# jafarinia/snuffy

Hardware: AMD Instinct MI355X
Metric: slides/sec (higher is better)
Workload: dtype f32; 1 GPU; cfgB: MILNet eval forward, 1 bag/step/rank, N=32768 patches D=768 h=6 Lambda=200 (K=200) depth=1 relu mlp x4; parallelism=bag-parallel x1, bags_resident_per_rank=8, launch=hip graph replay, rccl_ranks=0

## Files before the change

include/snuffy_hip.h:

```cpp
#ifndef SNUFFY_HIP_H
#define SNUFFY_HIP_H

#include <stddef.h>
#include <stdint.h>

#ifdef __cplusplus
extern "C" {
#endif

typedef void* snf_stream_t;

#define SNF_OK 0
#define SNF_EINVAL (-1)
#define SNF_ELAUNCH (-2)
#define SNF_EUNSUPPORTED (-3)
#define SNF_EWORKSPACE (-4)

#define SNF_ACT_RELU 0
#define SNF_ACT_GELU 1
#define SNF_ACT_LEAKYRELU 2
#define SNF_ACT_SELU 3
#define SNF_ACT_NONE 4

#define SNF_DT_F32 0
// ... 3 lines not shown

const char* snf_version(void);
const char* snf_last_error(void);
int snf_device_cu_count(void);

int snf_critic_f32(const float* x, int64_t n, int d, const float* w, const float* b, int c_out, float* scores,
                   float* colmax_val, int64_t* colmax_idx, snf_stream_t stream);
int snf_critic_ln_f32(const float* x, int64_t n, int d, const float* w, const float* b, int c_out, float* scores,
                      float eps, void* xhat_bf16, snf_stream_t stream);

#define SNF_TOPK_MAX_K 2048
size_t snf_topk_workspace_bytes(int64_t n, int k);
int snf_topk_f32(const float* scores, int64_t n, int64_t stride, int k, int64_t* idx_out, void* workspace,
                 size_t workspace_bytes, snf_stream_t stream);
int snf_topk_gather_f32(const float* scores, int64_t n, int64_t stride, int k, int64_t* idx_out, const float* x,
                        int d, float* xs, void* workspace, size_t workspace_bytes, snf_stream_t stream);
int snf_gather_rows_f32(const float* x, int64_t n, int d, const int64_t* idx, int k, float* out,
                        snf_stream_t stream);

size_t snf_selector_state_bytes(void);
int snf_critic_select_f32(const float* x, int64_t n, int d, const float* w, const float* b, float* scores, float eps,
                          void* xhat_bf16, void* selector_state, snf_stream_t stream);
int snf_topk_select_f32(const float* scores, int64_t n, int k, int64_t* idx_out, void* selector_state,
                        snf_stream_t stream);
int snf_topk_hist_select_f32(const float* scores, int64_t n, int64_t stride, int k, int64_t* idx_out, void* state,
                             snf_stream_t stream);

int snf_scatter_rows_f32(const float* x, int64_t n, int d, const int64_t* idx, int k, const float* rows, float* y,
                         snf_stream_t stream);
int snf_scatter_add_rows_f32(float* z, int64_t n, int d, const int64_t* idx, int k, const float* delta,
                             snf_stream_t stream);
int snf_slot_map_i32(const int64_t* idx, int k, int64_t n, int32_t* map, snf_stream_t stream);
int snf_gather_slot_map_f32(const float* x, int64_t n, int d, const int64_t* idx, int k, float* xs, int32_t* map,
                            void* xs_bf16, snf_stream_t stream);

int snf_layernorm_rows_f32(const float* x, int64_t n, int d, const int32_t* slot_map, const float* patch_rows,
                           const float* gamma, const float* beta, float eps, float* out_f32, void* out_bf16,
                           float* mean, float* rstd, const int64_t* out_row_idx, snf_stream_t stream);
int snf_layernorm_bwd_blocks(int64_t n);
int snf_layernorm_rows_bwd_f32(const float* x, int64_t n, int d, const void* dy, int dy_dtype, int64_t dy_stride,
                               const float* gamma, float eps, const float* residual, float* dx, void* dx_bf16,
                               float* partials, snf_stream_t stream);
int snf_fold_blocks(int r);
int snf_fold_linear_f32(const float* w, int r, int c, const float* gamma, const float* beta, const float* bias, void* wf_bf16,
                        int64_t ldwf, float* bf_f32, void* bf_bf16, snf_stream_t stream);
int snf_unfold_linear_f32(const float* dwf, const float* w, int r, int c, const float* gamma, const float* beta, const float* dbf,
                          float* dw, float* partial, snf_stream_t stream);
int snf_split3_f32(const float* x, int64_t ldx, int64_t m, int k, void* out_bf16, snf_stream_t stream);
int snf_mil_loss_f32(const float* ins, int64_t n, int c, const float* logits, const float* label, const float* w, const float* pos_weight,
                     const float* weight, float* out, int64_t* argmax, snf_stream_t stream);
int snf_mil_loss_bwd_f32(const float* grad_out, const float* fwd_out, const int64_t* argmax, int64_t n, int c, float* d_ins, float* d_small,
                         snf_stream_t stream);
int snf_split3_weight_f32(const float* w, int64_t ldw, int64_t m, int k, const float* colscale, void* out_bf16, snf_stream_t stream);
int snf_colsum_blocks(int64_t n);
int snf_colsum_fused(const void* src, int src_dtype, int64_t n, int d, const float* row_weight, int64_t weight_stride,
                     const void* gate_bf16, void* dst_bf16, float* partial, snf_stream_t stream);
int snf_dropout_rows_bf16(void* x, int64_t ldx, int64_t m, int n, float dropout_p, uint64_t seed, uint64_t offset, snf_stream_t stream);
int snf_residual_assemble_dropout_f32(const float* x, int64_t n, int d, const void* add_bf16, const float* add_bias,
                                      const int32_t* slot_map, const float* delta_rows, float dropout_p, uint64_t seed, uint64_t offset,
                                      float* z_out, snf_stream_t stream);
int snf_colsum_fused_dropout(const void* src, int src_dtype, int64_t n, int d, float dropout_p, uint64_t seed, uint64_t offset,
                             void* dst_bf16, float* partial, snf_stream_t stream);
int snf_split3_colsum_f32(const float* x, int64_t ldx, int64_t m, int k, const void* gate_bf16, int64_t ldg, void* out_bf16,
                          int64_t ldo, int64_t plane, float* partial, snf_stream_t stream);
int snf_split_hl_colsum_f32(const float* x, int64_t ldx, int64_t m, int k, const void* gate_hl, int64_t ldg, void* out_hl, int64_t ldo,
                            float* partial, snf_stream_t stream);
int snf_linear_rows_x3_f32(const float* x, int64_t ldx, const float* w, int64_t ldw, const float* bias, int r, int c, int k, void* out,
                           int64_t ldo, int out_dtype, snf_stream_t stream);
int snf_linear_rows_x3_resid_f32(const float* x, int64_t ldx, const float* w, int64_t ldw, const float* bias, const float* resid, int64_t ldr,
                                 int r, int c, int k, float* out, int64_t ldo, float* out2, int64_t ldo2, snf_stream_t stream);
int snf_critic_ln_hl_f32(const float* x, int64_t n, int d, const float* w, const float* b, int c_out, float* scores,
                         const float* gamma, const float* beta, float eps, void* out_hl, void* selector_state,
                         snf_stream_t stream);
int snf_layernorm_rows_split3_f32(const float* x, int64_t n, int d, const int32_t* slot_map, const float* patch_rows,
                                  const float* gamma, const float* beta, float eps, void* out_bf16, snf_stream_t stream);

int snf_bias_act(void* h, int dtype, int64_t n, int f, const float* bias, int act, snf_stream_t stream);

size_t snf_ln_mean_head_workspace_bytes(int d);
int snf_ln_mean_head_f32(const float* z, int64_t n, int d, const void* add_bf16, const float* add_bias,
                         const int32_t* slot_map, const float* delta_rows, float* z_out, const float* gamma,
                         const float* beta, float eps, const float* w_head, const float* b_head, int c_out,
                         float* logits, float* pooled, void* workspace, size_t workspace_bytes, snf_stream_t stream);

size_t snf_sparse_attn_fwd_workspace_bytes(int64_t n, int k, int h, int dk, int mfma);
int snf_sparse_attn_fwd_f32(const float* q, const float* kp, const float* v, int64_t n, int k, int h, int dk,
                            float scale, float* out, float* attn, float* lse, void* workspace,
                            size_t workspace_bytes, snf_stream_t stream);
int snf_sparse_attn_fwd_x3u_f32(const float* q, int64_t ldq, const float* kp, const float* v, int64_t ldv, int64_t n, int k, int h, int dk,
                                float scale, float* out, float* attn, float* lse, void* workspace, size_t workspace_bytes,
                                snf_stream_t stream);
int snf_sparse_attn_fwd_mfma(const void* q, int64_t ldq, const void* v, int64_t ldv, int qv_dtype, const void* kp,
                             int kp_dtype, int64_t n, int k, int h, int dk, float scale, float* out, float* attn,
                             float* lse, void* workspace, size_t workspace_bytes, snf_stream_t stream);

int snf_sparse_attn_fwd_mfma_dropout(const void* q, int64_t ldq, const void* v, int64_t ldv, int qv_dtype, const void* kp,
                                     int kp_dtype, int64_t n, int k, int h, int dk, float scale, float* out, float* attn,
                                     float* lse, float dropout_p, uint64_t seed, uint64_t offset, void* workspace,
                                     size_t workspace_bytes, snf_stream_t stream);
int snf_sparse_attn_bwd_mfma_dropout(const void* q, int64_t ldq, const void* v, int64_t ldv, int qv_dtype, const float* kp,
                                     const float* dout, const float* lse, const float* mask, float dropout_p, uint64_t seed,
                                     uint64_t offset, int64_t n, int k, int h, int dk, float scale, float* dq, float* dv,
                                     void* ds, int ds_dtype, snf_stream_t stream);
int snf_dropout_mask_f32(float dropout_p, uint64_t seed, uint64_t offset, int h, int64_t n, int k, float* mask,
                         snf_stream_t stream);

size_t snf_sparse_attn_fwd_x3_workspace_bytes(int64_t n, int k, int h, int dk);
int snf_sparse_attn_fwd_x3(const float* q, int64_t ldq, const float* v, int64_t ldv, const float* kp, int64_t n, int k, int h,
                           int dk, float scale, float* out, float* attn, float* lse, void* workspace, size_t workspace_bytes,
                           snf_stream_t stream);
int snf_sparse_attn_fwd_x3_dropout(const float* q, int64_t ldq, const float* v, int64_t ldv, const float* kp, int64_t n, int k, int h,
                                   int dk, float scale, float dropout_p, uint64_t seed, uint64_t offset, float* out, float* attn,
                                   float* lse, void* workspace, size_t workspace_bytes, snf_stream_t stream);

size_t snf_sparse_attn_fwd_x3_hl_workspace_bytes(int64_t n, int k, int h, int dk);
int snf_sparse_attn_fwd_x3_hl(const void* q_hl, int64_t ldq, const void* v_hl, int64_t ldv, const float* kp, int64_t n, int k, int h,
                              int dk, float scale, float* out, float* attn, float* lse, void* workspace, size_t workspace_bytes,
                              snf_stream_t stream);
size_t snf_sparse_attn_x3_hl_kpfrag_bytes(int k, int h, int dk);
int snf_linear_rows_x3_kpfrag_f32(const float* x, int64_t ldx, const float* w, int64_t ldw, const float* bias, int k_keys, int h, int dk,
                                  int kdim, float scale, void* kp_frag, size_t kp_frag_bytes, snf_stream_t stream);
int snf_gather_linear_rows_x3_kpfrag_f32(const float* x, int64_t ldx, int64_t n, const int64_t* idx, const float* w, int64_t ldw,
                                         const float* bias, int k_keys, int h, int dk, int kdim, float scale, void* kp_frag,
                                         size_t kp_frag_bytes, float* xs, int32_t* slot_map, snf_stream_t stream);
int snf_sparse_attn_fwd_x3_hl_kpfrag(const void* q_hl, int64_t ldq, const void* v_hl, int64_t ldv, const void* kp_frag, int64_t n, int k,
                                     int h, int dk, float* out, float* attn, float* lse, void* workspace, size_t workspace_bytes,
                                     snf_stream_t stream);

size_t snf_sparse_attn_bwd_workspace_bytes(int64_t n, int k, int h, int dk);
int snf_sparse_attn_bwd_f32(const float* q, const float* kp, const float* v, const float* p, const float* mask,
                            const float* dout, int64_t n, int k, int h, int dk, float scale, float* dq, float* dkp,
                            float* dv, void* workspace, size_t workspace_bytes, snf_stream_t stream);
int snf_sparse_attn_bwd_ld_f32(const float* q, int64_t ldq, const float* kp, const float* v, int64_t ldv, const float* p, const float* mask,
                               const float* dout, int64_t n, int k, int h, int dk, float scale, float* dq, float* dkp, float* dv,
                               void* workspace, size_t workspace_bytes, snf_stream_t stream);
int snf_sparse_attn_bwd_dropout_f32(const float* q, int64_t ldq, const float* kp, const float* v, int64_t ldv, const float* p, float dropout_p,
                                    uint64_t seed, uint64_t offset, const float* dout, int64_t n, int k, int h, int dk, float scale, float* dq,
                                    float* dkp, float* dv, void* workspace, size_t workspace_bytes, snf_stream_t stream);
int snf_sparse_attn_bwd_mfma(const void* q, int64_t ldq, const void* v, int64_t ldv, int qv_dtype, const float* kp,
                             const float* dout, const float* lse, const float* mask, int64_t n, int k, int h, int dk,
                             float scale, float* dq, float* dv, void* ds, int ds_dtype, snf_stream_t stream);
int snf_sparse_attn_bwd_mfma_ex(const void* q, int64_t ldq, const void* v, int64_t ldv, int qv_dtype, const float* kp,
                                const float* dout, const float* lse, const float* mask, float dropout_p, uint64_t seed,
                                uint64_t offset, int64_t n, int k, int h, int dk, float scale, void* dq, void* dv, int64_t ldd,
                                int dqv_dtype, void* ds, int ds_dtype, snf_stream_t stream);
size_t snf_sparse_attn_bwd_mfma_chunked_workspace_bytes(int64_t n, int k, int h, int dk, int dqv_dtype);
int snf_sparse_attn_bwd_mfma_chunked(const void* q, int64_t ldq, const void* v, int64_t ldv, int qv_dtype, const float* kp,
                                     const float* dout, const float* lse, const float* mask, float dropout_p, uint64_t seed,
                                     uint64_t offset, int64_t n, int k, int h, int dk, float scale, void* dq, void* dv, int64_t ldd,
                                     int dqv_dtype, void* ds, int ds_dtype, void* workspace, size_t workspace_bytes,
                                     snf_stream_t stream);
int snf_sparse_attn_dkp_f32(const float* ds, const float* q, int64_t n, int k, int h, int dk, float* dkp, void* workspace,
                            size_t workspace_bytes, snf_stream_t stream);

int snf_gemm_bf16(const void* a, int64_t lda, const void* w, int64_t ldw, const float* bias, int64_t m, int n, int k,
                  int act, void* c, int64_t ldc, int out_dtype, int tile_n, snf_stream_t stream);
int snf_gemm_bf16_dropout(const void* a, int64_t lda, const void* w, int64_t ldw, const float* bias, int64_t m, int n, int k, int act,
                          void* c, int64_t ldc, int out_dtype, int tile_n, float dropout_p, uint64_t seed, uint64_t offset,
                          snf_stream_t stream);
int snf_gemm_bf16_resid_f32(const void* a, int64_t lda, const void* w, int64_t ldw, const float* bias, const float* resid, int64_t ldr,
                            int64_t m, int n, int k, int act, float* c, int64_t ldc, int tile_n, snf_stream_t stream);
int snf_gemm_bf16_lnfold(const void* a, int64_t lda, const void* w, int64_t ldw, const float* colsum, const float* bias,
                         const float* rowstats, int64_t m, int n, int k, int act, void* c, int64_t ldc, snf_stream_t stream);
int snf_gemm_bf16_resid(const void* a, int64_t lda, const void* w, int64_t ldw, const float* bias, int64_t m, int n, int k, float* x,
                        int64_t ldx, void* x_bf16, int64_t ldxb, float* stats_part, snf_stream_t stream);
int snf_gemm_hl_bf16(const void* a_hl, int64_t lda, const void* w_hl, int64_t ldw, const float* bias, int64_t m, int n, int k,
                     int act, void* c, int64_t ldc, int out_dtype, snf_stream_t stream);
int snf_gemm_hl_resid_bf16(const void* a_hl, int64_t lda, const void* w_hl, int64_t ldw, const float* bias, const float* resid,
                           int64_t ldr, int64_t m, int n, int k, int act, void* c, int64_t ldc, int out_dtype, snf_stream_t stream);
size_t snf_gemm_hl_ws_bytes(int64_t m, int n, int k);
int snf_gemm_hl_gated_bf16(const void* a_hl, int64_t lda, const void* w_hl, int64_t ldw, const void* gate_hl, int64_t ldg, int64_t m, int n,
                           int k, void* c_hl, int64_t ldc, snf_stream_t stream);
size_t snf_gemm_tn_ws_bytes(int64_t n, int p, int q);
int snf_gemm_tn_f32(const void* a, int64_t lda, int a_hi, int a_lo, const void* b, int64_t ldb, int b_hi, int b_lo, int hl, int64_t n, int p,
                    int q, float* c, int64_t ldc, void* workspace, size_t workspace_bytes, snf_stream_t stream);
int snf_gemm_hl_ws_bf16(const void* a_hl, int64_t lda, const void* w_hl, int64_t ldw, const float* bias, const float* resid,
                        int64_t ldr, int64_t m, int n, int k, int act, void* c, int64_t ldc, int out_dtype, void* workspace,
                        size_t workspace_bytes, snf_stream_t stream);
int snf_gemm_hl_dropout_bf16(const void* a_hl, int64_t lda, const void* w_hl, int64_t ldw, const float* bias, const float* resid,
                             int64_t ldr, int64_t m, int n, int k, int act, void* c, int64_t ldc, int out_dtype, float dropout_p,
                             uint64_t seed, uint64_t offset, snf_stream_t stream);
int snf_gemm_hl_ws_dropout_bf16(const void* a_hl, int64_t lda, const void* w_hl, int64_t ldw, const float* bias, const float* resid,
                                int64_t ldr, int64_t m, int n, int k, int act, void* c, int64_t ldc, int out_dtype, float dropout_p,
                                uint64_t seed, uint64_t offset, void* workspace, size_t workspace_bytes, snf_stream_t stream);
int snf_split_hl_colsum_dropout_f32(const float* x, int64_t ldx, int64_t m, int k, const void* gate_hl, int64_t ldg, float dropout_p,
                                    uint64_t seed, uint64_t offset, void* out_hl, int64_t ldo, float* partial, snf_stream_t stream);
int snf_split_hl_f32(const float* x, int64_t ldx, int64_t m, int k, void* out_bf16, snf_stream_t stream);
int snf_layernorm_rows_hl_f32(const float* x, int64_t n, int d, const int32_t* slot_map, const float* patch_rows,
                              const float* gamma, const float* beta, float eps, void* out_bf16, snf_stream_t stream);
int snf_layernorm_rows_hl_patch_f32(const float* x, const float* addend, int64_t n, int d, const int64_t* out_row_idx,
                                    const float* gamma, const float* beta, float eps, void* out_hl, snf_stream_t stream);

int snf_vit_patchify(const float* img, int b, int c, int hgt, int wid, int patch, void* cols, int out_dtype,
                     snf_stream_t stream);
int snf_vit_assemble_tokens(const void* patch_emb, int pe_dtype, const float* cls_token, const float* pos_embed, int b,
                            int num_patches, int d, float* tokens, snf_stream_t stream);
int snf_vit_residual_ln(float* x, int64_t n, int d, const void* add1_bf16, const void* add2_bf16, float scale2,
                        const float* gamma, const float* beta, float eps, void* ln_out_bf16, void* x_bf16,
                        snf_stream_t stream);
int snf_vit_row_stats(const float* x, int64_t ldx, const float* part, int slots, int64_t n, int d, float eps, float* stats,
                      void* x_bf16, int64_t ldxb, snf_stream_t stream);
int snf_vit_attention_f32(const float* qkv, int b, int t, int h, int dk, float scale, float* out, float* attn,
                          snf_stream_t stream);
#define SNF_VIT_MFMA_MAX_T 4096
int snf_vit_attention_mfma(const void* qkv_bf16, int b, int t, int h, int dk, float scale, void* out_bf16,
                           snf_stream_t stream);
int snf_vit_attention_x3_f32(const float* qkv, int b, int t, int h, int dk, float scale, void* out, int out_dtype, snf_stream_t stream);

int snf_tile_preprocess_u8(const void* img_u8, int b, int h, int w, int c, int oh, int ow, const int* hbounds, const int* hcoef,
                           int hks, const int* vbounds, const int* vcoef, int vks, int normalize, const float* mean,
                           const float* std_, float* out_f32, void* cols_bf16, int patch, snf_stream_t stream);

int snf_topk_segmented_f32(const float* scores, const int64_t* offsets_dev, int bags, int64_t max_n, int k, int64_t* idx_out,
                           snf_stream_t stream);
int snf_sparse_attn_varlen_plan(const int64_t* offsets, int bags, int k, int h, int dk, int32_t* table, size_t table_ints,
                                size_t* table_ints_needed, size_t* workspace_bytes);
int snf_sparse_attn_fwd_mfma_varlen(const void* q, int64_t ldq, const void* v, int64_t ldv, const void* kp, int kp_dtype,
                                    const int64_t* offsets, int bags, int k, int h, int dk, float scale, float* out, float* attn,
                                    float* lse, const int32_t* table_dev, void* workspace, size_t workspace_bytes,
                                    snf_stream_t stream);
int snf_sparse_attn_x3_varlen_plan(const int64_t* offsets, int bags, int k, int h, int dk, int32_t* table, size_t table_ints,
                                   size_t* table_ints_needed, size_t* workspace_bytes);
int snf_sparse_attn_fwd_x3_varlen(const float* q, int64_t ldq, const float* v, int64_t ldv, const float* kp, const int64_t* offsets,
                                  int bags, int k, int h, int dk, float scale, float* out, float* attn, float* lse,
                                  const int32_t* table_dev, void* workspace, size_t workspace_bytes, snf_stream_t stream);
int snf_sparse_attn_varlen_chunked_plan(const int64_t* offsets, int bags, int k, int h, int dk, int32_t* table, size_t table_ints,
                                        size_t* table_ints_needed, size_t* workspace_bytes, int* n_chunks, int* chunk_k);
int snf_sparse_attn_fwd_mfma_varlen_chunked(const void* q, int64_t ldq, const void* v, int64_t ldv, const void* kp, int kp_dtype,
                                            const int64_t* offsets, int bags, int k, int h, int dk, float scale, float* out,
                                            float* attn, float* lse, const int32_t* table_dev, void* workspace,
                                            size_t workspace_bytes, snf_stream_t stream);
int snf_sparse_attn_x3_varlen_chunked_plan(const int64_t* offsets, int bags, int k, int h, int dk, int32_t* table, size_t table_ints,
                                           size_t* table_ints_needed, size_t* workspace_bytes, int* n_chunks, int* chunk_k);
int snf_sparse_attn_fwd_x3_varlen_chunked(const float* q, int64_t ldq, const float* v, int64_t ldv, const float* kp,
                                          const int64_t* offsets, int bags, int k, int h, int dk, float scale, float* out, float* attn,
                                          float* lse, const int32_t* table_dev, void* workspace, size_t workspace_bytes,
                                          snf_stream_t stream);
int snf_sparse_attn_fwd_ragged_f32(const float* q, int64_t ldq, const float* v, int64_t ldv, const float* kp, const int32_t* desc_dev,
                                   int bags, int64_t n_total, int kmax, int h, int dk, float scale, float* out, float* attn,
                                   float* lse, snf_stream_t stream);
int snf_ln_mean_head_varlen_plan(const int64_t* offsets, int bags, int d, int32_t* table, size_t table_ints,
                                 size_t* table_ints_needed, size_t* workspace_bytes);
int snf_ln_mean_head_varlen_f32(const float* z, const int64_t* offsets, int bags, int d, const void* add_bf16,
                                const float* add_bias, const int32_t* slot_map, const float* delta_rows, float* z_out,
                                const float* gamma, const float* beta, float eps, const float* w_head, const float* b_head,
                                int c_out, float* logits, float* pooled, const int32_t* table_dev, void* workspace,
                                size_t workspace_bytes, snf_stream_t stream);

int snf_sampler_advance(void* state, snf_stream_t stream);
int snf_random_share_keys_f32(const void* state, int layer, int64_t n, const int64_t* exclude_rows, int n_exclude, float* keys,
                              snf_stream_t stream);

void snf_debug_attn_trace(void* buf);
void snf_debug_attn_trace_wg(int wg);
void snf_debug_x3p_kbw(int kbw);
void snf_debug_exact_attn_mfma(int on);

#ifdef __cplusplus
}
#endif
#endif
// ... 1 lines not shown
```

snuffy_amd/_ffi.py:

```python
import ctypes
import os
from ctypes import c_char_p, c_float, c_int, c_int64, c_size_t, c_uint64, c_void_p

_HERE = os.path.dirname(os.path.abspath(__file__))
LIB_PATH = os.environ.get("SNUFFY_HIP_LIB") or os.path.join(_HERE, "lib", "libsnuffy_hip.so")

SNF_OK = 0
SNF_EINVAL = -1
SNF_ELAUNCH = -2
SNF_EUNSUPPORTED = -3
SNF_EWORKSPACE = -4

ACT_CODES = {"relu": 0, "gelu": 1, "leakyrelu": 2, "selu": 3, "none": 4}
DT_F32 = 0
DT_BF16 = 1
DT_BF16_SPLIT3 = 2
DT_BF16_HL = 3
TOPK_MAX_K = 2048

SIGNATURES = {
    "snf_version": (c_char_p, []),
    "snf_last_error": (c_char_p, []),
    "snf_device_cu_count": (c_int, []),
    "snf_critic_f32": (c_int, [c_void_p, c_int64, c_int, c_void_p, c_void_p, c_int, c_void_p, c_void_p, c_void_p,
                               c_void_p]),
    "snf_critic_ln_f32": (c_int, [c_void_p, c_int64, c_int, c_void_p, c_void_p, c_int, c_void_p, c_float, c_void_p,
                                  c_void_p]),
    "snf_topk_workspace_bytes": (c_size_t, [c_int64, c_int]),
    "snf_topk_f32": (c_int, [c_void_p, c_int64, c_int64, c_int, c_void_p, c_void_p, c_size_t, c_void_p]),
    "snf_topk_gather_f32": (c_int, [c_void_p, c_int64, c_int64, c_int, c_void_p, c_void_p, c_int, c_void_p, c_void_p,
                                    c_size_t, c_void_p]),
    "snf_gather_rows_f32": (c_int, [c_void_p, c_int64, c_int, c_void_p, c_int, c_void_p, c_void_p]),
    "snf_selector_state_bytes": (c_size_t, []),
    "snf_critic_select_f32": (c_int, [c_void_p, c_int64, c_int, c_void_p, c_void_p, c_void_p, c_float, c_void_p, c_void_p,
                                      c_void_p]),
    "snf_topk_select_f32": (c_int, [c_void_p, c_int64, c_int, c_void_p, c_void_p, c_void_p]),
    "snf_topk_hist_select_f32": (c_int, [c_void_p, c_int64, c_int64, c_int, c_void_p, c_void_p, c_void_p]),
    "snf_scatter_rows_f32": (c_int, [c_void_p, c_int64, c_int, c_void_p, c_int, c_void_p, c_void_p, c_void_p]),
    "snf_scatter_add_rows_f32": (c_int, [c_void_p, c_int64, c_int, c_void_p, c_int, c_void_p, c_void_p]),
    "snf_slot_map_i32": (c_int, [c_void_p, c_int, c_int64, c_void_p, c_void_p]),
    "snf_gather_slot_map_f32": (c_int, [c_void_p, c_int64, c_int, c_void_p, c_int, c_void_p, c_void_p, c_void_p, c_void_p]),
    "snf_layernorm_rows_f32": (c_int, [c_void_p, c_int64, c_int, c_void_p, c_void_p, c_void_p, c_void_p, c_float,
                                       c_void_p, c_void_p, c_void_p, c_void_p, c_void_p, c_void_p]),
    "snf_layernorm_bwd_blocks": (c_int, [c_int64]),
    "snf_layernorm_rows_bwd_f32": (c_int, [c_void_p, c_int64, c_int, c_void_p, c_int, c_int64, c_void_p, c_float, c_void_p,
                                           c_void_p, c_void_p, c_void_p, c_void_p]),
    "snf_fold_blocks": (c_int, [c_int]),
    "snf_fold_linear_f32": (c_int, [c_void_p, c_int, c_int, c_void_p, c_void_p, c_void_p, c_void_p, c_int64, c_void_p, c_void_p,
                                    c_void_p]),
    "snf_unfold_linear_f32": (c_int, [c_void_p, c_void_p, c_int, c_int, c_void_p, c_void_p, c_void_p, c_void_p, c_void_p,
                                      c_void_p]),
    "snf_split3_f32": (c_int, [c_void_p, c_int64, c_int64, c_int, c_void_p, c_void_p]),
    "snf_mil_loss_f32": (c_int, [c_void_p, c_int64, c_int, c_void_p, c_void_p, c_void_p, c_void_p, c_void_p, c_void_p, c_void_p, c_void_p]),
    "snf_mil_loss_bwd_f32": (c_int, [c_void_p, c_void_p, c_void_p, c_int64, c_int, c_void_p, c_void_p, c_void_p]),
    "snf_split3_weight_f32": (c_int, [c_void_p, c_int64, c_int64, c_int, c_void_p, c_void_p, c_void_p]),
    "snf_split3_colsum_f32": (c_int, [c_void_p, c_int64, c_int64, c_int, c_void_p, c_int64, c_void_p, c_int64, c_int64, c_void_p, c_void_p]),
    "snf_colsum_blocks": (c_int, [c_int64]),
    "snf_colsum_fused": (c_int, [c_void_p, c_int, c_int64, c_int, c_void_p, c_int64, c_void_p, c_void_p, c_void_p, c_void_p]),
    "snf_layernorm_rows_split3_f32": (c_int, [c_void_p, c_int64, c_int, c_void_p, c_void_p, c_void_p, c_void_p, c_float,
                                              c_void_p, c_void_p]),
    "snf_linear_rows_x3_f32": (c_int, [c_void_p, c_int64, c_void_p, c_int64, c_void_p, c_int, c_int, c_int, c_void_p, c_int64, c_int,
                                       c_void_p]),
    "snf_critic_ln_hl_f32": (c_int, [c_void_p, c_int64, c_int, c_void_p, c_void_p, c_int, c_void_p, c_void_p, c_void_p, c_float,
                                     c_void_p, c_void_p, c_void_p]),
    "snf_bias_act": (c_int, [c_void_p, c_int, c_int64, c_int, c_void_p, c_int, c_void_p]),
    "snf_ln_mean_head_workspace_bytes": (c_size_t, [c_int]),
    "snf_ln_mean_head_f32": (c_int, [c_void_p, c_int64, c_int, c_void_p, c_void_p, c_void_p, c_void_p, c_void_p,
                                     c_void_p, c_void_p, c_float, c_void_p, c_void_p, c_int, c_void_p, c_void_p,
                                     c_void_p, c_size_t, c_void_p]),
    "snf_sparse_attn_fwd_workspace_bytes": (c_size_t, [c_int64, c_int, c_int, c_int, c_int]),
    "snf_sparse_attn_fwd_f32": (c_int, [c_void_p, c_void_p, c_void_p, c_int64, c_int, c_int, c_int, c_float, c_void_p,
                                        c_void_p, c_void_p, c_void_p, c_size_t, c_void_p]),
    "snf_sparse_attn_fwd_x3u_f32": (c_int, [c_void_p, c_int64, c_void_p, c_void_p, c_int64, c_int64, c_int, c_int, c_int, c_float, c_void_p,
                                            c_void_p, c_void_p, c_void_p, c_size_t, c_void_p]),
    "snf_sparse_attn_bwd_workspace_bytes": (c_size_t, [c_int64, c_int, c_int, c_int]),
    "snf_sparse_attn_bwd_f32": (c_int, [c_void_p, c_void_p, c_void_p, c_void_p, c_void_p, c_void_p, c_int64, c_int, c_int,
                                        c_int, c_float, c_void_p, c_void_p, c_void_p, c_void_p, c_size_t, c_void_p]),
    "snf_sparse_attn_bwd_ld_f32": (c_int, [c_void_p, c_int64, c_void_p, c_void_p, c_int64, c_void_p, c_void_p, c_void_p, c_int64, c_int, c_int,
                                           c_int, c_float, c_void_p, c_void_p, c_void_p, c_void_p, c_size_t, c_void_p]),
    "snf_sparse_attn_bwd_dropout_f32": (c_int, [c_void_p, c_int64, c_void_p, c_void_p, c_int64, c_void_p, c_float, c_uint64, c_uint64, c_void_p,
                                                c_int64, c_int, c_int, c_int, c_float, c_void_p, c_void_p, c_void_p, c_void_p, c_size_t, c_void_p]),
    "snf_sparse_attn_bwd_mfma": (c_int, [c_void_p, c_int64, c_void_p, c_int64, c_int, c_void_p, c_void_p, c_void_p, c_void_p,
                                         c_int64, c_int, c_int, c_int, c_float, c_void_p, c_void_p, c_void_p, c_int, c_void_p]),
    "snf_sparse_attn_dkp_f32": (c_int, [c_void_p, c_void_p, c_int64, c_int, c_int, c_int, c_void_p, c_void_p, c_size_t,
                                        c_void_p]),
    "snf_sparse_attn_fwd_mfma": (c_int, [c_void_p, c_int64, c_void_p, c_int64, c_int, c_void_p, c_int, c_int64, c_int, c_int,
                                         c_int, c_float, c_void_p, c_void_p, c_void_p, c_void_p, c_size_t, c_void_p]),
    "snf_sparse_attn_fwd_x3_workspace_bytes": (c_size_t, [c_int64, c_int, c_int, c_int]),
    "snf_sparse_attn_fwd_x3": (c_int, [c_void_p, c_int64, c_void_p, c_int64, c_void_p, c_int64, c_int, c_int, c_int, c_float,
                                       c_void_p, c_void_p, c_void_p, c_void_p, c_size_t, c_void_p]),
    "snf_sparse_attn_fwd_x3_dropout": (c_int, [c_void_p, c_int64, c_void_p, c_int64, c_void_p, c_int64, c_int, c_int, c_int, c_float,
                                               c_float, c_uint64, c_uint64, c_void_p, c_void_p, c_void_p, c_void_p, c_size_t, c_void_p]),
    "snf_sparse_attn_fwd_x3_hl_workspace_bytes": (c_size_t, [c_int64, c_int, c_int, c_int]),
    "snf_sparse_attn_x3_hl_kpfrag_bytes": (c_size_t, [c_int, c_int, c_int]),
    "snf_linear_rows_x3_kpfrag_f32": (c_int, [c_void_p, c_int64, c_void_p, c_int64, c_void_p, c_int, c_int, c_int, c_int, c_float,
                                              c_void_p, c_size_t, c_void_p]),
    "snf_gather_linear_rows_x3_kpfrag_f32": (c_int, [c_void_p, c_int64, c_int64, c_void_p, c_void_p, c_int64, c_void_p, c_int, c_int, c_int,
                                                     c_int, c_float, c_void_p, c_size_t, c_void_p, c_void_p, c_void_p]),
    "snf_sparse_attn_fwd_x3_hl_kpfrag": (c_int, [c_void_p, c_int64, c_void_p, c_int64, c_void_p, c_int64, c_int, c_int, c_int,
                                                 c_void_p, c_void_p, c_void_p, c_void_p, c_size_t, c_void_p]),
    "snf_sparse_attn_fwd_x3_hl": (c_int, [c_void_p, c_int64, c_void_p, c_int64, c_void_p, c_int64, c_int, c_int, c_int, c_float,
                                          c_void_p, c_void_p, c_void_p, c_void_p, c_size_t, c_void_p]),
    "snf_sparse_attn_fwd_mfma_dropout": (c_int, [c_void_p, c_int64, c_void_p, c_int64, c_int, c_void_p, c_int, c_int64, c_int, c_int,
                                                 c_int, c_float, c_void_p, c_void_p, c_void_p, c_float, c_uint64, c_uint64,
                                                 c_void_p, c_size_t, c_void_p]),
    "snf_sparse_attn_bwd_mfma_dropout": (c_int, [c_void_p, c_int64, c_void_p, c_int64, c_int, c_void_p, c_void_p, c_void_p, c_void_p,
                                                 c_float, c_uint64, c_uint64, c_int64, c_int, c_int, c_int, c_float, c_void_p,
                                                 c_void_p, c_void_p, c_int, c_void_p]),
    "snf_sparse_attn_bwd_mfma_ex": (c_int, [c_void_p, c_int64, c_void_p, c_int64, c_int, c_void_p, c_void_p, c_void_p, c_void_p,
                                            c_float, c_uint64, c_uint64, c_int64, c_int, c_int, c_int, c_float, c_void_p,
                                            c_void_p, c_int64, c_int, c_void_p, c_int, c_void_p]),
    "snf_sparse_attn_bwd_mfma_chunked_workspace_bytes": (c_size_t, [c_int64, c_int, c_int, c_int, c_int]),
    "snf_sparse_attn_bwd_mfma_chunked": (c_int, [c_void_p, c_int64, c_void_p, c_int64, c_int, c_void_p, c_void_p, c_void_p, c_void_p,
                                                 c_float, c_uint64, c_uint64, c_int64, c_int, c_int, c_int, c_float, c_void_p,
                                                 c_void_p, c_int64, c_int, c_void_p, c_int, c_void_p, c_size_t, c_void_p]),
    "snf_dropout_mask_f32": (c_int, [c_float, c_uint64, c_uint64, c_int, c_int64, c_int, c_void_p, c_void_p]),
    "snf_tile_preprocess_u8": (c_int, [c_void_p, c_int, c_int, c_int, c_int, c_int, c_int, c_void_p, c_void_p, c_int, c_void_p,
                                       c_void_p, c_int, c_int, c_void_p, c_void_p, c_void_p, c_void_p, c_int, c_void_p]),
    "snf_gemm_bf16": (c_int, [c_void_p, c_int64, c_void_p, c_int64, c_void_p, c_int64, c_int, c_int, c_int, c_void_p, c_int64,
                              c_int, c_int, c_void_p]),
    "snf_gemm_bf16_resid_f32": (c_int, [c_void_p, c_int64, c_void_p, c_int64, c_void_p, c_void_p, c_int64, c_int64, c_int, c_int, c_int,
                                        c_void_p, c_int64, c_int, c_void_p]),
    "snf_linear_rows_x3_resid_f32": (c_int, [c_void_p, c_int64, c_void_p, c_int64, c_void_p, c_void_p, c_int64, c_int, c_int, c_int,
                                             c_void_p, c_int64, c_void_p, c_int64, c_void_p]),
    "snf_gemm_bf16_lnfold": (c_int, [c_void_p, c_int64, c_void_p, c_int64, c_void_p, c_void_p, c_void_p, c_int64, c_int, c_int, c_int,
                                     c_void_p, c_int64, c_void_p]),
    "snf_gemm_bf16_resid": (c_int, [c_void_p, c_int64, c_void_p, c_int64, c_void_p, c_int64, c_int, c_int, c_void_p, c_int64, c_void_p,
                                    c_int64, c_void_p, c_void_p]),
    "snf_vit_row_stats": (c_int, [c_void_p, c_int64, c_void_p, c_int, c_int64, c_int, c_float, c_void_p, c_void_p, c_int64, c_void_p]),
    "snf_split_hl_f32": (c_int, [c_void_p, c_int64, c_int64, c_int, c_void_p, c_void_p]),
    "snf_layernorm_rows_hl_patch_f32": (c_int, [c_void_p, c_void_p, c_int64, c_int, c_void_p, c_void_p, c_void_p, c_float, c_void_p,
                                                c_void_p]),
    "snf_layernorm_rows_hl_f32": (c_int, [c_void_p, c_int64, c_int, c_void_p, c_void_p, c_void_p, c_void_p, c_float,
                                          c_void_p, c_void_p]),
    "snf_gemm_hl_resid_bf16": (c_int, [c_void_p, c_int64, c_void_p, c_int64, c_void_p, c_void_p, c_int64, c_int64, c_int, c_int, c_int,
                                       c_void_p, c_int64, c_int, c_void_p]),
    "snf_gemm_hl_ws_bytes": (c_size_t, [c_int64, c_int, c_int]),
    "snf_gemm_hl_gated_bf16": (c_int, [c_void_p, c_int64, c_void_p, c_int64, c_void_p, c_int64, c_int64, c_int, c_int, c_void_p, c_int64,
                                       c_void_p]),
    "snf_gemm_tn_ws_bytes": (c_size_t, [c_int64, c_int, c_int]),
    "snf_gemm_tn_f32": (c_int, [c_void_p, c_int64, c_int, c_int, c_void_p, c_int64, c_int, c_int, c_int, c_int64, c_int, c_int, c_void_p,
                                c_int64, c_void_p, c_size_t, c_void_p]),
    "snf_split_hl_colsum_f32": (c_int, [c_void_p, c_int64, c_int64, c_int, c_void_p, c_int64, c_void_p, c_int64, c_void_p, c_void_p]),
    "snf_gemm_hl_ws_bf16": (c_int, [c_void_p, c_int64, c_void_p, c_int64, c_void_p, c_void_p, c_int64, c_int64, c_int, c_int, c_int,
                                    c_void_p, c_int64, c_int, c_void_p, c_size_t, c_void_p]),
    "snf_gemm_bf16_dropout": (c_int, [c_void_p, c_int64, c_void_p, c_int64, c_void_p, c_int64, c_int, c_int, c_int, c_void_p, c_int64,
                                      c_int, c_int, c_float, c_uint64, c_uint64, c_void_p]),
    "snf_dropout_rows_bf16": (c_int, [c_void_p, c_int64, c_int64, c_int, c_float, c_uint64, c_uint64, c_void_p]),
    "snf_residual_assemble_dropout_f32": (c_int, [c_void_p, c_int64, c_int, c_void_p, c_void_p, c_void_p, c_void_p, c_float, c_uint64,
                                                  c_uint64, c_void_p, c_void_p]),
    "snf_colsum_fused_dropout": (c_int, [c_void_p, c_int, c_int64, c_int, c_float, c_uint64, c_uint64, c_void_p, c_void_p, c_void_p]),
    "snf_gemm_hl_dropout_bf16": (c_int, [c_void_p, c_int64, c_void_p, c_int64, c_void_p, c_void_p, c_int64, c_int64, c_int, c_int, c_int,
                                         c_void_p, c_int64, c_int, c_float, c_uint64, c_uint64, c_void_p]),
    "snf_gemm_hl_ws_dropout_bf16": (c_int, [c_void_p, c_int64, c_void_p, c_int64, c_void_p, c_void_p, c_int64, c_int64, c_int, c_int, c_int,
                                            c_void_p, c_int64, c_int, c_float, c_uint64, c_uint64, c_void_p, c_size_t, c_void_p]),
    "snf_split_hl_colsum_dropout_f32": (c_int, [c_void_p, c_int64, c_int64, c_int, c_void_p, c_int64, c_float, c_uint64, c_uint64,
                                                c_void_p, c_int64, c_void_p, c_void_p]),
    "snf_gemm_hl_bf16": (c_int, [c_void_p, c_int64, c_void_p, c_int64, c_void_p, c_int64, c_int, c_int, c_int, c_void_p, c_int64,
                                 c_int, c_void_p]),
    "snf_topk_segmented_f32": (c_int, [c_void_p, c_void_p, c_int, c_int64, c_int, c_void_p, c_void_p]),
    "snf_sparse_attn_varlen_plan": (c_int, [c_void_p, c_int, c_int, c_int, c_int, c_void_p, c_size_t, c_void_p, c_void_p]),
    "snf_sparse_attn_fwd_mfma_varlen": (c_int, [c_void_p, c_int64, c_void_p, c_int64, c_void_p, c_int, c_void_p, c_int, c_int, c_int,
                                                c_int, c_float, c_void_p, c_void_p, c_void_p, c_void_p, c_void_p, c_size_t,
                                                c_void_p]),
    "snf_sparse_attn_x3_varlen_plan": (c_int, [c_void_p, c_int, c_int, c_int, c_int, c_void_p, c_size_t, c_void_p, c_void_p]),
    "snf_sparse_attn_fwd_x3_varlen": (c_int, [c_void_p, c_int64, c_void_p, c_int64, c_void_p, c_void_p, c_int, c_int, c_int, c_int,
                                              c_float, c_void_p, c_void_p, c_void_p, c_void_p, c_void_p, c_size_t, c_void_p]),
    "snf_sparse_attn_varlen_chunked_plan": (c_int, [c_void_p, c_int, c_int, c_int, c_int, c_void_p, c_size_t, c_void_p, c_void_p,
                                                    c_void_p, c_void_p]),
    "snf_sparse_attn_fwd_mfma_varlen_chunked": (c_int, [c_void_p, c_int64, c_void_p, c_int64, c_void_p, c_int, c_void_p, c_int, c_int,
                                                        c_int, c_int, c_float, c_void_p, c_void_p, c_void_p, c_void_p, c_void_p,
                                                        c_size_t, c_void_p]),
    "snf_sparse_attn_x3_varlen_chunked_plan": (c_int, [c_void_p, c_int, c_int, c_int, c_int, c_void_p, c_size_t, c_void_p, c_void_p,
                                                       c_void_p, c_void_p]),
    "snf_sparse_attn_fwd_x3_varlen_chunked": (c_int, [c_void_p, c_int64, c_void_p, c_int64, c_void_p, c_void_p, c_int, c_int, c_int,
                                                      c_int, c_float, c_void_p, c_void_p, c_void_p, c_void_p, c_void_p, c_size_t,
                                                      c_void_p]),
    "snf_sparse_attn_fwd_ragged_f32": (c_int, [c_void_p, c_int64, c_void_p, c_int64, c_void_p, c_void_p, c_int, c_int64, c_int, c_int,
                                               c_int, c_float, c_void_p, c_void_p, c_void_p, c_void_p]),
    "snf_ln_mean_head_varlen_plan": (c_int, [c_void_p, c_int, c_int, c_void_p, c_size_t, c_void_p, c_void_p]),
    "snf_ln_mean_head_varlen_f32": (c_int, [c_void_p, c_void_p, c_int, c_int, c_void_p, c_void_p, c_void_p, c_void_p, c_void_p,
                                            c_void_p, c_void_p, c_float, c_void_p, c_void_p, c_int, c_void_p, c_void_p, c_void_p,
                                            c_void_p, c_size_t, c_void_p]),
    "snf_vit_patchify": (c_int, [c_void_p, c_int, c_int, c_int, c_int, c_int, c_void_p, c_int, c_void_p]),
    "snf_vit_assemble_tokens": (c_int, [c_void_p, c_int, c_void_p, c_void_p, c_int, c_int, c_int, c_void_p, c_void_p]),
    "snf_vit_residual_ln": (c_int, [c_void_p, c_int64, c_int, c_void_p, c_void_p, c_float, c_void_p, c_void_p, c_float,
                                    c_void_p, c_void_p, c_void_p]),
    "snf_vit_attention_f32": (c_int, [c_void_p, c_int, c_int, c_int, c_int, c_float, c_void_p, c_void_p, c_void_p]),
    "snf_sampler_advance": (c_int, [c_void_p, c_void_p]),
    "snf_random_share_keys_f32": (c_int, [c_void_p, c_int, c_int64, c_void_p, c_int, c_void_p, c_void_p]),
    "snf_debug_attn_trace": (None, [c_void_p]),
    "snf_debug_attn_trace_wg": (None, [c_int]),
    "snf_debug_x3p_kbw": (None, [c_int]),
    "snf_debug_exact_attn_mfma": (None, [c_int]),
    "snf_vit_attention_mfma": (c_int, [c_void_p, c_int, c_int, c_int, c_int, c_float, c_void_p, c_void_p]),
    "snf_vit_attention_x3_f32": (c_int, [c_void_p, c_int, c_int, c_int, c_int, c_float, c_void_p, c_int, c_void_p]),
}

_lib = None


class SnuffyHipError(RuntimeError):
    pass


def load():
    global _lib
    if _lib is not None:
        return _lib
    if not os.path.exists(LIB_PATH):
        raise SnuffyHipError(
            "libsnuffy_hip.so not found at %s -- build it with `python -m snuffy_amd.build` "
            "(or __graft_entry__.build()); there is no CPU fallback" % LIB_PATH)
    import torch
    lib = ctypes.CDLL(LIB_PATH)
    for name, (res, args) in SIGNATURES.items():
        fn = getattr(lib, name)
        fn.restype = res
        fn.argtypes = args
    _lib = lib
    return lib


def check(rc, what):
    if rc != SNF_OK:
        msg = load().snf_last_error()
        raise SnuffyHipError("%s failed (code %d): %s" % (what, rc, msg.decode() if msg else "?"))

# ... 4 lines not shown
```

snuffy_amd/csrc/gemm.hip:

```cpp
#include <stdlib.h>

#include "mfma.h"
#include "philox.h"

namespace {

struct GemmParams {
    const unsigned short* a;
    const unsigned short* w;
    const float* bias;
    void* c;
    int64_t lda, ldw, ldc;
    int m, n, k;
    int act;
    int tiles_m, tiles_n;
    unsigned long long* trace;
    const float* resid = nullptr;
    int64_t ldr = 0;
    unsigned int* split_cnt = nullptr;
    float* split_slab = nullptr;
    int split_cap = 0, split_rcap = 0;
    const unsigned short* gate = nullptr;
    int64_t ldg = 0;
    const float* colsum = nullptr;
// ... 374 lines not shown
#pragma unroll
                for (int h = 0; h < NI / 2; ++h) {
                    s1[h] += __shfl_xor(s1[h], 16, 64), s2[h] += __shfl_xor(s2[h], 16, 64);
                    s1[h] += __shfl_xor(s1[h], 32, 64), s2[h] += __shfl_xor(s2[h], 32, 64);
                }
                if constexpr (NI == 4) {
                    const int g = 2 * (WC * tn + wc);
                    if (fg == 0 && (FULL || (g < P.slots && row < P.m)))
                        *reinterpret_cast<f32x4*>(P.stats_part + 2 * ((int64_t)row * P.slots + g)) = f32x4{s1[0], s2[0], s1[1], s2[1]};
                } else {
                    const int g = 4 * tn + wc;
                    if (fg == 0 && (FULL || (g < P.slots && row < P.m)))
                        *reinterpret_cast<f32x2*>(P.stats_part + 2 * ((int64_t)row * P.slots + g)) = f32x2{s1[0], s2[0]};
                }
            }
        }
    };

    Src cur = tile_src(tile);
#pragma unroll
    for (int i = 0; i < AHEAD; ++i) stage(cur, i, i);
    wait_vmcnt<(AHEAD - 1) * GL>();
    __builtin_amdgcn_s_barrier();
    __builtin_amdgcn_sched_barrier(0);
    if (wid >= 4) __builtin_amdgcn_s_barrier();

    int rb = 0, sb = AHEAD;
    bool after_epilogue = false;
    while (true) {
        const int next = tile + wgs_per_xcd;
        const bool has_next = next < t_hi;
        const Src nxt = tile_src(has_next ? next : tile);
        const bool full = (tile / P.tiles_n + 1) * BM <= P.m && (tile % P.tiles_n + 1) * BN <= P.n;
        for (int s = 0; s < ns; ++s) {
            if constexpr (EPI == 2)
                if (s == 0) preload_x(tile);
            read_frags(rb);
            if (s == ns - 1) load_bias(tile);
            const bool in_tile = s + AHEAD < ns;
            const int exist = has_next ? AHEAD : (ns - 1 - s < AHEAD ? ns - 1 - s : AHEAD);
            if (in_tile)
                stage(cur, s + AHEAD, sb);
            else if (has_next)
                stage(nxt, s + AHEAD - ns, sb);
            if (exist == AHEAD) {
                if (after_epilogue)
                    wait_vmcnt<(AHEAD - 1) * GL + MI * NST>();
                else
                    wait_vmcnt<(AHEAD - 1) * GL>();
            } else if (AHEAD == 3 && exist == 2) {
                wait_vmcnt<GL>();
            } else {
                wait_vmcnt<0>();
            }
            after_epilogue = false;
            rb = rb == NBUF - 1 ? 0 : rb + 1;
            sb = sb == NBUF - 1 ? 0 : sb + 1;
            barrier();
            if (s == 0)
                mma(std::true_type{});
            else
                mma(std::false_type{});
            barrier();
        }
        bias_landed();
#ifdef SNF_GEMM_NOSTORE
        if (false) {
#else
        if (full) {
#endif
            epilogue(tile, std::true_type{});
            after_epilogue = true;
        } else {
            epilogue(tile, std::false_type{});
            wait_vmcnt<0>();
        }
        if (!has_next) break;
        tile = next;
        cur = nxt;
    }
    if (wid < 4) __builtin_amdgcn_s_barrier();
}

template <int ACT, int OUT, bool SPLIT = false, bool GATE = false, bool DROP = false>
__global__ __launch_bounds__(512, 2) void gemm_hl_kernel(GemmParams P) {
    static_assert(!GATE || (OUT == 3 && ACT == SNF_ACT_NONE && !SPLIT), "gemm_hl: the gated form writes an hl image, no activation, no split");
    static_assert(!DROP || (!GATE && (OUT == 1 || OUT == 3)), "gemm_hl: dropout goes with the fp32 and the hl-image outputs");
    constexpr int NI = 4, BN = 256;
    constexpr int ROWL = 128;
    constexpr int IMG = BM * ROWL;
    constexpr int STEP_BYTES = 2 * IMG;
    constexpr int NC = 4 * NI;
    constexpr bool LINE_STORES = (OUT == 1 || OUT == 3) && ACT != SNF_ACT_GELU && ACT != SNF_ACT_SELU;
    extern __shared__ __attribute__((aligned(16))) unsigned char smem[];

    const int lane = threadIdx.x & 63;
    const int wid = __builtin_amdgcn_readfirstlane(threadIdx.x >> 6);
    const int wr = wid >> 2, wc = wid & 3;
    const int ns_all = P.k / BKS;
    unsigned char* const scr = smem + 2 * STEP_BYTES + wid * 4096;

    const int ntiles = P.tiles_m * P.tiles_n;
    const int xcd = blockIdx.x & 7, wg_in_xcd = blockIdx.x >> 3, wgs_per_xcd = gridDim.x >> 3;
    if constexpr (!SPLIT) {
        if (P.split_cap >= 2 && blockIdx.x == 0) {
            for (int i = threadIdx.x; i < 8 * P.split_rcap; i += 512) P.split_cnt[i] = 0u;
            asm volatile("s_waitcnt vmcnt(0)" ::: "memory");
        }
    }
    int t_lo, t_hi;
    {
        const int q = ntiles >> 3, r = ntiles & 7;
        t_lo = xcd < r ? xcd * (q + 1) : r * (q + 1) + (xcd - r) * q;
        t_hi = t_lo + q + (xcd < r ? 1 : 0);
    }
    int sp_part = 0, sp_parts = 1, sp_slot = 0, sp_tile = -1;
    if (P.split_cap >= 2) {
        const int q_x = t_hi - t_lo, full_rounds = q_x / wgs_per_xcd, r = q_x - full_rounds * wgs_per_xcd;
        int sn = r > 0 ? wgs_per_xcd / r : 0;
        if (sn > P.split_cap) sn = P.split_cap;
        if (sn > ns_all / HL_SPLIT_MIN_STEPS) sn = ns_all / HL_SPLIT_MIN_STEPS;
        if (sn >= 2 && r <= P.split_rcap) {
            if constexpr (SPLIT) {
                if (wg_in_xcd < r * sn) {
                    const int jr = wg_in_xcd % r;
                    sp_tile = t_lo + full_rounds * wgs_per_xcd + jr;
                    sp_part = wg_in_xcd / r, sp_parts = sn, sp_slot = xcd * P.split_rcap + jr;
                }
            } else {
                t_hi = t_lo + full_rounds * wgs_per_xcd;
            }
        }
    }
    int tile = t_lo + wg_in_xcd;
    if constexpr (SPLIT) {
        tile = __builtin_amdgcn_readfirstlane(sp_tile);
        sp_part = __builtin_amdgcn_readfirstlane(sp_part), sp_parts = __builtin_amdgcn_readfirstlane(sp_parts);
        sp_slot = __builtin_amdgcn_readfirstlane(sp_slot);
        if (tile < 0) return;
        t_hi = tile + 1;
        asm volatile("" : "+s"(t_hi));
    } else {
        if (tile >= t_hi) return;
    }
    const int s_begin = SPLIT ? __builtin_amdgcn_readfirstlane(sp_part * ns_all / sp_parts) : 0;
    const int ns = SPLIT ? __builtin_amdgcn_readfirstlane((sp_part + 1) * ns_all / sp_parts) - s_begin : ns_all;
    const unsigned short* const a_base = P.a + (SPLIT ? s_begin * 64 : 0);
    const unsigned short* const w_base = P.w + (SPLIT ? s_begin * 64 : 0);

    struct Src {
        int a[4], w[4];
    };
    auto tile_src_mn = [&](int tm, int tn) __attribute__((always_inline)) -> Src {
        Src s;
        int ln = lane;
        asm volatile("" : "+v"(ln));
        const int c = ln & 7;
#pragma unroll
        for (int j = 0; j < 4; ++j) {
            const int row = (4 * wid + j) * 8 + (ln >> 3);
            int grow = tm * BM + row;
            if (grow > P.m - 1) grow = P.m - 1;
            s.a[j] = grow * (int)P.lda + ((c ^ ((row >> 1) & 7)) << 3);
            int wrow = tn * BN + row;
            if (wrow > P.n - 1) wrow = P.n - 1;
            s.w[j] = wrow * (int)P.ldw + ((c ^ (((row >> 1) & 1) | (((row >> 3) & 3) << 1))) << 3);
        }
        return s;
// ... 135 lines not shown
                            *reinterpret_cast<u32x4*>(dst + 32) = pl;
                        }
                    }
                }
            }
            if constexpr (LINE_STORES) {
                const int lr = lane_o >> 4, lc = lane_o & 15;
                unsigned char* const crow = reinterpret_cast<unsigned char*>(P.c) +
                                            (OUT == 1 ? 4 * (int64_t)(tn * BN + 64 * wc) : 2 * 2 * (int64_t)(tn * BN + 64 * wc));
                const int64_t pitch = (OUT == 1 ? 4 : 2) * P.ldc;
#pragma unroll
                for (int jj = 0; jj < 4; ++jj) {
                    const int r = lr + 4 * jj;
                    const u32x4 val = *reinterpret_cast<const u32x4*>(scr + r * 256 + ((lc ^ r) << 4));
                    const int orow = tm * BM + 128 * wr + 16 * mi + r;
                    const int ocol = tn * BN + 64 * wc + (OUT == 1 ? 4 * lc : 32 * (lc >> 3) + 8 * (lc & 3));
#ifdef X3_NOSTORE
                    const bool ok2 = val[0] == 0x12345678u && orow < 0;
#else
                    const bool ok2 = FULL || (orow < P.m && ocol + (OUT == 1 ? 4 : 8) <= P.n);
#endif
                    if (ok2) *reinterpret_cast<u32x4*>(crow + orow * pitch + 16 * lc) = val;
                }
            }
        }
    };

    Src cur = tile_src(tile);
    stage(cur, 0, 0);
    int buf = 0;
    bool after_epilogue = false;
    while (true) {
        const int next = tile + wgs_per_xcd;
        const bool has_next = next < t_hi;
        const bool full = (tile / P.tiles_n + 1) * BM <= P.m && (tile % P.tiles_n + 1) * BN <= P.n;
        for (int s = 0; s < ns; ++s) {
            if (!(s == 0 && after_epilogue)) wait_vmcnt<0>();
            after_epilogue = false;
            __builtin_amdgcn_sched_barrier(0);
            __builtin_amdgcn_s_barrier();
            __builtin_amdgcn_sched_barrier(0);
            const unsigned char* base = smem + buf * STEP_BYTES;
#pragma unroll
            for (int ni = 0; ni < NI; ++ni) wh[ni] = frag(base + woff_h + (4 * (ni & 1) + 32 * (ni >> 1)) * ROWL);
#pragma unroll
            for (int mi = 0; mi < 8; ++mi) xf[mi] = frag(base + xoff_h + mi * 16 * ROWL);
#pragma unroll
            for (int ni = 0; ni < NI; ++ni) wl[ni] = frag(base + woff_l + (4 * (ni & 1) + 32 * (ni >> 1)) * ROWL);
            __builtin_amdgcn_sched_barrier(0);
            if (s + 1 < ns) {
                stage(cur, s + 1, buf ^ 1);
            } else if (has_next) {
                cur = tile_src(next);
                stage(cur, 0, buf ^ 1);
            }
            __builtin_amdgcn_sched_barrier(0);
            __builtin_amdgcn_s_setprio(1);
            if (s == 0) {
#pragma unroll
                for (int mi = 0; mi < 8; ++mi)
#pragma unroll
                    for (int ni = 0; ni < NI; ++ni) acc[mi][ni] = X3_MFMA(wh[ni], xf[mi], (f32x4{0.f, 0.f, 0.f, 0.f}));
            } else {
#pragma unroll
                for (int mi = 0; mi < 8; ++mi)
#pragma unroll
                    for (int ni = 0; ni < NI; ++ni) acc[mi][ni] = X3_MFMA(wh[ni], xf[mi], acc[mi][ni]);
            }
#pragma unroll
            for (int mi = 0; mi < 8; ++mi) {
#pragma unroll
                for (int ni = 0; ni < NI; ++ni) acc[mi][ni] = X3_MFMA(wl[ni], xf[mi], acc[mi][ni]);
                __builtin_amdgcn_sched_barrier(0);
                xf[mi] = frag(base + xoff_l + mi * 16 * ROWL);
                __builtin_amdgcn_sched_barrier(0);
            }
#pragma unroll
            for (int mi = 0; mi < 8; ++mi)
#pragma unroll
                for (int ni = 0; ni < NI; ++ni) acc[mi][ni] = X3_MFMA(wh[ni], xf[mi], acc[mi][ni]);
            __builtin_amdgcn_s_setprio(0);
            buf ^= 1;
        }
        if constexpr (SPLIT) {
            volatile unsigned int& s_ticket = *reinterpret_cast<volatile unsigned int*>(smem);
            float* slab0 = P.split_slab + (size_t)sp_slot * P.split_cap * (size_t)(BM * BN);
            unsigned tix = threadIdx.x;
            asm volatile("" : "+v"(tix));
            f32x4* mine = reinterpret_cast<f32x4*>(slab0 + (size_t)sp_part * (BM * BN)) + tix;
            wait_vmcnt<0>();
#pragma unroll
            for (int mi = 0; mi < 8; ++mi)
#pragma unroll
                for (int ni = 0; ni < NI; ++ni) mine[(mi * NI + ni) * 512] = acc[mi][ni];
            wait_vmcnt<0>();
            __syncthreads();
            if (tix == 0) {
                __builtin_amdgcn_fence(__ATOMIC_RELEASE, "agent");
                asm volatile("s_waitcnt vmcnt(0)" ::: "memory");
                s_ticket = __hip_atomic_fetch_add(P.split_cnt + sp_slot, 1u, __ATOMIC_RELAXED, __HIP_MEMORY_SCOPE_AGENT);
            }
            __syncthreads();
            if (s_ticket != (unsigned)(sp_parts - 1)) return;
            __syncthreads();
            if (tix == 0) {
                __builtin_amdgcn_fence(__ATOMIC_ACQUIRE, "agent");
                __hip_atomic_store(P.split_cnt + sp_slot, 0u, __ATOMIC_RELAXED, __HIP_MEMORY_SCOPE_AGENT);
            }
            __syncthreads();
#pragma unroll
            for (int mi = 0; mi < 8; ++mi)
#pragma unroll
                for (int ni = 0; ni < NI; ++ni) {
                    f32x4 sum = {0.f, 0.f, 0.f, 0.f};
                    for (int pp = 0; pp < sp_parts; ++pp) {
                        f32x4 v = acc[mi][ni];
                        if (pp != sp_part) v = reinterpret_cast<const f32x4*>(slab0 + (size_t)pp * (BM * BN))[(mi * NI + ni) * 512 + tix];
                        sum = pp == 0 ? v : sum + v;
                    }
                    acc[mi][ni] = sum;
                }
        }
        load_bias(tile);
        wait_vmcnt<0>();
        bias_landed();
        if (full)
            epilogue(tile, std::true_type{});
        else
            epilogue(tile, std::false_type{});
        after_epilogue = true;
        if (!has_next) break;
        tile = next;
    }
}

template <int ACT, int OUT, bool DROP = false>
int launch_hl(const GemmParams& P, hipStream_t s) {
    constexpr int lds = 2 * 2 * BM * 128 + (((OUT == 1 || OUT == 3) && ACT != SNF_ACT_GELU && ACT != SNF_ACT_SELU) ? 8 * 4096 : 0);
    auto kern = [] {
        if constexpr (DROP) return gemm_hl_kernel<ACT, OUT, false, false, true>;
        else return gemm_hl_kernel<ACT, OUT>;
    }();
    static thread_local unsigned long long attr_set_mask = 0;
    if (int rc = snf::lds_opt_in(reinterpret_cast<const void*>(kern), lds, &attr_set_mask, "gemm_hl")) return rc;
    const int ntiles = P.tiles_m * P.tiles_n;
    int grid = snf::cu_count() & ~7;
    if (grid < 8) grid = 8;
    {
        static const int dbg_grid = getenv("SNF_GEMM_HL_GRID") ? atoi(getenv("SNF_GEMM_HL_GRID")) & ~7 : 0;
        if (dbg_grid >= 8 && dbg_grid < grid && P.split_cap < 2) grid = dbg_grid;
    }
    const int per_xcd = (ntiles + 7) / 8;
    if (per_xcd * 8 < grid) grid = per_xcd * 8;
    hipLaunchKernelGGL(kern, dim3(grid), dim3(512), lds, s, P);
    int rc = snf::check_launch("gemm_hl_kernel");
    if (rc || P.split_cap < 2) return rc;
    auto kern2 = [] {
        if constexpr (DROP) return gemm_hl_kernel<ACT, OUT, true, false, true>;
        else return gemm_hl_kernel<ACT, OUT, true>;
    }();
    static thread_local unsigned long long attr_set2_mask = 0;
    if (int rc = snf::lds_opt_in(reinterpret_cast<const void*>(kern2), lds, &attr_set2_mask, "gemm_hl")) return rc;
    hipLaunchKernelGGL(kern2, dim3(grid), dim3(512), lds, s, P);
    return snf::check_launch("gemm_hl_kernel<split>");
}

int launch_hl_gated(const GemmParams& P, hipStream_t s) {
    constexpr int lds = 2 * 2 * BM * 128 + 8 * 4096;
    auto kern = gemm_hl_kernel<SNF_ACT_NONE, 3, false, true>;
    static thread_local unsigned long long attr_set_mask = 0;
    if (int rc = snf::lds_opt_in(reinterpret_cast<const void*>(kern), lds, &attr_set_mask, "gemm_hl")) return rc;
    const int ntiles = P.tiles_m * P.tiles_n;
    int grid = snf::cu_count() & ~7;
    if (grid < 8) grid = 8;
    const int per_xcd = (ntiles + 7) / 8;
    if (per_xcd * 8 < grid) grid = per_xcd * 8;
    hipLaunchKernelGGL(kern, dim3(grid), dim3(512), lds, s, P);
    return snf::check_launch("gemm_hl_kernel<gated>");
}

template <int OUT>
int launch_hl_act(const GemmParams& P, hipStream_t s) {
    switch (P.act) {
        case SNF_ACT_RELU: return launch_hl<SNF_ACT_RELU, OUT>(P, s);
        case SNF_ACT_GELU: return launch_hl<SNF_ACT_GELU, OUT>(P, s);
        case SNF_ACT_LEAKYRELU: return launch_hl<SNF_ACT_LEAKYRELU, OUT>(P, s);
        case SNF_ACT_SELU: return launch_hl<SNF_ACT_SELU, OUT>(P, s);
        default: return launch_hl<SNF_ACT_NONE, OUT>(P, s);
    }
}

template <int NI, int ACT, int OUT, int EPI = 0, int MI = 8, bool DROP = false>
int launch(const GemmParams& P, hipStream_t s) {
    constexpr int lds = NBUF * (A_BYTES + (MI == 8 ? 64 : 32) * NI * ROWB) +
                        ((EPI == 2 || (OUT == 0 && NI == 4 && ACT != SNF_ACT_GELU && ACT != SNF_ACT_SELU)) ? 8 * 4096 : 0);
    auto kern = [] {
        if constexpr (DROP) return gemm_bf16_kernel<NI, ACT, OUT, EPI, MI, true>;
        else return gemm_bf16_kernel<NI, ACT, OUT, EPI, MI>;
    }();
    static thread_local unsigned long long attr_set_mask = 0;
    if (int rc = snf::lds_opt_in(reinterpret_cast<const void*>(kern), lds, &attr_set_mask, "gemm_bf16")) return rc;
    const int ntiles = P.tiles_m * P.tiles_n;
    int grid = snf::cu_count() & ~7;
    if (grid < 8) grid = 8;
    const int per_xcd = (ntiles + 7) / 8;
    if (per_xcd * 8 < grid) grid = per_xcd * 8;
    hipLaunchKernelGGL(kern, dim3(grid), dim3(512), lds, s, P);
    return snf::check_launch("gemm_bf16_kernel");
}

#ifndef SNF_GEMM_128_MI4
#define SNF_GEMM_128_MI4 1
// ... 344 lines not shown
    return g;
}
constexpr size_t HL_TICKET_BYTES = 4096;
}

extern "C" size_t snf_gemm_hl_ws_bytes(int64_t m, int n, int k) {
    const HlSplit g = hl_split_geometry(m, n, k);
    if (g.cap < 2 || 8 * g.rcap * sizeof(unsigned int) > HL_TICKET_BYTES) return 0;
    return HL_TICKET_BYTES + (size_t)8 * g.rcap * g.cap * (size_t)(BM * 256) * sizeof(float);
}

extern "C" int snf_gemm_hl_resid_bf16(const void* a_hl, int64_t lda, const void* w_hl, int64_t ldw, const float* bias,
                                      const float* resid, int64_t ldr, int64_t m, int n, int k, int act, void* c, int64_t ldc,
                                      int out_dtype, snf_stream_t stream) {
    return snf_gemm_hl_ws_bf16(a_hl, lda, w_hl, ldw, bias, resid, ldr, m, n, k, act, c, ldc, out_dtype, nullptr, 0, stream);
}

namespace {
int gemm_hl_ws_impl(const void* a_hl, int64_t lda, const void* w_hl, int64_t ldw, const float* bias, const float* resid, int64_t ldr,
                    int64_t m, int n, int k, int act, void* c, int64_t ldc, int out_dtype, const snf::DropoutState* drop, void* workspace,
                    size_t workspace_bytes, snf_stream_t stream) {
    SNF_REQUIRE(a_hl && w_hl && c, "snf_gemm_hl_bf16: null pointer");
    SNF_REQUIRE(m >= 1 && n >= 1 && k >= 1, "snf_gemm_hl_bf16: bad shape m=%lld n=%d k=%d", (long long)m, n, k);
    SNF_REQUIRE(act >= SNF_ACT_RELU && act <= SNF_ACT_NONE, "snf_gemm_hl_bf16: bad activation code %d", act);
    SNF_REQUIRE(out_dtype == SNF_DT_F32 || out_dtype == SNF_DT_BF16 || out_dtype == SNF_DT_BF16_HL,
                "snf_gemm_hl_bf16: bad output dtype %d", out_dtype);
    const bool hl_out = out_dtype == SNF_DT_BF16_HL;
    SNF_REQUIRE(!resid || (out_dtype == SNF_DT_F32 && ldr >= n && ldr % 4 == 0 && reinterpret_cast<uintptr_t>(resid) % 16 == 0),
                "snf_gemm_hl_bf16: a residual needs an fp32 output and 16-byte aligned rows (ldr=%lld)", (long long)ldr);
    if (k % BKS || k < BKS || n % 8 || (hl_out && n % 32) || lda % 8 || ldw % 8 || ldc % (out_dtype == SNF_DT_F32 ? 4 : 8) ||
        lda < 2 * (int64_t)k || ldw < 2 * (int64_t)k || ldc < (hl_out ? 2 * (int64_t)n : n) ||
        (reinterpret_cast<uintptr_t>(a_hl) | reinterpret_cast<uintptr_t>(w_hl) | reinterpret_cast<uintptr_t>(c)) % 16 ||
        (bias && reinterpret_cast<uintptr_t>(bias) % 16) || m * lda >= 0x7fffffffll || (int64_t)n * ldw >= 0x7fffffffll) {
        snf::set_error("snf_gemm_hl_bf16: shape m=%lld n=%d k=%d (lda %lld ldw %lld ldc %lld) outside the kernel's domain "
                       "(k %% 32, n %% 8 (%% 32 for an hl output), images of 2 k columns, 16-byte aligned rows, 31-bit element offsets)",
                       (long long)m, n, k, (long long)lda, (long long)ldw, (long long)ldc);
        return SNF_EUNSUPPORTED;
    }
    GemmParams P;
    P.a = reinterpret_cast<const unsigned short*>(a_hl);
    P.w = reinterpret_cast<const unsigned short*>(w_hl);
    P.bias = bias;
    P.c = c;
    P.lda = lda, P.ldw = ldw, P.ldc = ldc;
    P.m = (int)m, P.n = n, P.k = k, P.act = act;
    P.tiles_m = (int)((m + BM - 1) / BM);
    P.tiles_n = (n + 255) / 256;
    P.trace = nullptr;
    P.resid = resid;
    P.ldr = ldr;
    if (workspace) {
        const size_t need = snf_gemm_hl_ws_bytes(m, n, k);
        if (need) {
            if (workspace_bytes < need || reinterpret_cast<uintptr_t>(workspace) % 16) {
                snf::set_error("snf_gemm_hl_ws_bf16: workspace %zu < %zu (or not 16-byte aligned)", workspace_bytes, need);
                return SNF_EWORKSPACE;
            }
            const HlSplit g = hl_split_geometry(m, n, k);
            P.split_cnt = reinterpret_cast<unsigned int*>(workspace);
            P.split_slab = reinterpret_cast<float*>(reinterpret_cast<unsigned char*>(workspace) + HL_TICKET_BYTES);
            P.split_cap = g.cap, P.split_rcap = g.rcap;
        }
    }
    hipStream_t s = snf::as_stream(stream);
    if (drop && drop->thresh) {
        P.drop = *drop;
        if (hl_out && act == SNF_ACT_RELU && !resid) return launch_hl<SNF_ACT_RELU, 3, true>(P, s);
        if (out_dtype == SNF_DT_F32 && act == SNF_ACT_NONE) return launch_hl<SNF_ACT_NONE, 1, true>(P, s);
        snf::set_error("snf_gemm_hl_dropout_bf16: dropout exists for act = relu with an hl-image output and for act = none with an fp32 "
                       "output (got act %d, out_dtype %d)", act, out_dtype);
        return SNF_EUNSUPPORTED;
    }
    if (hl_out) return launch_hl_act<3>(P, s);
    return out_dtype == SNF_DT_F32 ? launch_hl_act<1>(P, s) : launch_hl_act<0>(P, s);
}
}

extern "C" int snf_gemm_hl_ws_bf16(const void* a_hl, int64_t lda, const void* w_hl, int64_t ldw, const float* bias,
                                   const float* resid, int64_t ldr, int64_t m, int n, int k, int act, void* c, int64_t ldc,
                                   int out_dtype, void* workspace, size_t workspace_bytes, snf_stream_t stream) {
    return gemm_hl_ws_impl(a_hl, lda, w_hl, ldw, bias, resid, ldr, m, n, k, act, c, ldc, out_dtype, nullptr, workspace, workspace_bytes, stream);
}

extern "C" int snf_gemm_hl_ws_dropout_bf16(const void* a_hl, int64_t lda, const void* w_hl, int64_t ldw, const float* bias,
                                           const float* resid, int64_t ldr, int64_t m, int n, int k, int act, void* c, int64_t ldc,
                                           int out_dtype, float dropout_p, uint64_t seed, uint64_t offset, void* workspace,
                                           size_t workspace_bytes, snf_stream_t stream) {
    SNF_REQUIRE(dropout_p >= 0.f && dropout_p < 1.f, "snf_gemm_hl_dropout_bf16: dropout_p=%f outside [0, 1)", dropout_p);
    const snf::DropoutState st = snf::make_dropout(dropout_p, seed, offset);
    return gemm_hl_ws_impl(a_hl, lda, w_hl, ldw, bias, resid, ldr, m, n, k, act, c, ldc, out_dtype, &st, workspace, workspace_bytes, stream);
}

extern "C" int snf_gemm_hl_dropout_bf16(const void* a_hl, int64_t lda, const void* w_hl, int64_t ldw, const float* bias,
                                        const float* resid, int64_t ldr, int64_t m, int n, int k, int act, void* c, int64_t ldc,
                                        int out_dtype, float dropout_p, uint64_t seed, uint64_t offset, snf_stream_t stream) {
    return snf_gemm_hl_ws_dropout_bf16(a_hl, lda, w_hl, ldw, bias, resid, ldr, m, n, k, act, c, ldc, out_dtype, dropout_p, seed, offset,
                                       nullptr, 0, stream);
}

extern "C" int snf_gemm_hl_gated_bf16(const void* a_hl, int64_t lda, const void* w_hl, int64_t ldw, const void* gate_hl, int64_t ldg, int64_t m,
                                      int n, int k, void* c_hl, int64_t ldc, snf_stream_t stream) {
    SNF_REQUIRE(a_hl && w_hl && gate_hl && c_hl, "snf_gemm_hl_gated_bf16: null pointer");
    SNF_REQUIRE(m >= 1 && n >= 1 && k >= 1, "snf_gemm_hl_gated_bf16: bad shape m=%lld n=%d k=%d", (long long)m, n, k);
    if (k % BKS || k < BKS || n % 32 || lda % 8 || ldw % 8 || ldc % 8 || ldg % 8 || lda < 2 * (int64_t)k || ldw < 2 * (int64_t)k ||
        ldc < 2 * (int64_t)n || ldg < 2 * (int64_t)n ||
        (reinterpret_cast<uintptr_t>(a_hl) | reinterpret_cast<uintptr_t>(w_hl) | reinterpret_cast<uintptr_t>(c_hl) |
         reinterpret_cast<uintptr_t>(gate_hl)) % 16 ||
        m * lda >= 0x7fffffffll || (int64_t)n * ldw >= 0x7fffffffll) {
        snf::set_error("snf_gemm_hl_gated_bf16: shape m=%lld n=%d k=%d (lda %lld ldw %lld ldc %lld ldg %lld) outside the kernel's domain "
                       "(k %% 32, n %% 32, images of 2 k / 2 n columns, 16-byte aligned rows, 31-bit element offsets)",
                       (long long)m, n, k, (long long)lda, (long long)ldw, (long long)ldc, (long long)ldg);
        return SNF_EUNSUPPORTED;
    }
    GemmParams P;
    P.a = reinterpret_cast<const unsigned short*>(a_hl);
    P.w = reinterpret_cast<const unsigned short*>(w_hl);
    P.bias = nullptr;
    P.c = c_hl;
    P.lda = lda, P.ldw = ldw, P.ldc = ldc;
    P.m = (int)m, P.n = n, P.k = k, P.act = SNF_ACT_NONE;
    P.tiles_m = (int)((m + BM - 1) / BM);
    P.tiles_n = (n + 255) / 256;
    P.trace = nullptr;
    P.gate = reinterpret_cast<const unsigned short*>(gate_hl), P.ldg = ldg;
    return launch_hl_gated(P, snf::as_stream(stream));
}

extern "C" int snf_linear_rows_x3_f32(const float* x, int64_t ldx, const float* w, int64_t ldw, const float* bias, int r, int c, int k,
                                      void* out, int64_t ldo, int out_dtype, snf_stream_t stream) {
    SNF_REQUIRE(x && w && out, "snf_linear_rows_x3_f32: null pointer");
    SNF_REQUIRE(r >= 1 && r <= 8192 && c >= 1 && k >= 16 && k % 16 == 0, "snf_linear_rows_x3_f32: bad shape r=%d c=%d k=%d "
                "(r <= 8192, k %% 16 == 0)", r, c, k);
    SNF_REQUIRE(out_dtype == SNF_DT_F32 || out_dtype == SNF_DT_BF16, "snf_linear_rows_x3_f32: bad out dtype %d", out_dtype);
    SNF_REQUIRE(ldx >= k && ldw >= k && ldo >= c && (ldx % 4) == 0 && (ldw % 4) == 0 &&
                    ((reinterpret_cast<uintptr_t>(x) | reinterpret_cast<uintptr_t>(w)) & 15) == 0,
                "snf_linear_rows_x3_f32: x / w rows must be 16-byte aligned");
    const dim3 grid((unsigned)((c + 31) / 32), (unsigned)((r + 31) / 32));
    hipStream_t s = snf::as_stream(stream);
    if (out_dtype == SNF_DT_BF16)
        hipLaunchKernelGGL(skinny_linear_x3_kernel<true>, grid, dim3(512), 0, s, x, ldx, w, ldw, bias, r, c, k, out, ldo);
    else
        hipLaunchKernelGGL(skinny_linear_x3_kernel<false>, grid, dim3(512), 0, s, x, ldx, w, ldw, bias, r, c, k, out, ldo);
    return snf::check_launch("skinny_linear_x3_kernel");
}

extern "C" int snf_linear_rows_x3_resid_f32(const float* x, int64_t ldx, const float* w, int64_t ldw, const float* bias, const float* resid,
                                            int64_t ldr, int r, int c, int k, float* out, int64_t ldo, float* out2, int64_t ldo2,
                                            snf_stream_t stream) {
    SNF_REQUIRE(x && w && out && out2 && resid, "snf_linear_rows_x3_resid_f32: null pointer");
    SNF_REQUIRE(r >= 1 && r <= 8192 && c >= 1 && k >= 16 && k % 16 == 0, "snf_linear_rows_x3_resid_f32: bad shape r=%d c=%d k=%d "
                "(r <= 8192, k %% 16 == 0)", r, c, k);
    SNF_REQUIRE(ldx >= k && ldw >= k && ldo >= c && ldo2 >= c && ldr >= c && (ldx % 4) == 0 && (ldw % 4) == 0 &&
                    ((reinterpret_cast<uintptr_t>(x) | reinterpret_cast<uintptr_t>(w)) & 15) == 0,
                "snf_linear_rows_x3_resid_f32: x / w rows must be 16-byte aligned");
    const dim3 grid((unsigned)((c + 31) / 32), (unsigned)((r + 31) / 32));
    SkinnyFrag fr;
    fr.resid = resid, fr.ldr = ldr, fr.out2 = out2, fr.ldo2 = ldo2;
    hipLaunchKernelGGL(skinny_linear_x3_kernel<false>, grid, dim3(512), 0, snf::as_stream(stream), x, ldx, w, ldw, bias, r, c, k, out, ldo, fr);
    return snf::check_launch("skinny_linear_x3_kernel");
}
```

snuffy_amd/csrc/rowops.hip:

```cpp
#include <math.h>

#include "common.h"
#include "philox.h"
#include "selector.h"

namespace {

constexpr int WG = 256;
constexpr int WAVES = WG / 64;

template <int VEC>
struct VecT;
template <>
struct VecT<4> {
    using type = float4;
};
template <>
struct VecT<1> {
    using type = float;
};

template <int VEC, int NV>
struct RowRegs {
    float v[NV * VEC];
// ... 967 lines not shown
            return scale * (v > 0.f ? v : alpha * expm1f(v));
        }
        default:
            return v;
    }
}

__global__ __launch_bounds__(WG) void bias_act_f32_kernel(float* __restrict__ h, int64_t n, int f,
                                                          const float* __restrict__ bias, int act) {
    const int64_t total = n * (int64_t)f;
    if ((f & 3) == 0) {
        for (int64_t i4 = ((int64_t)blockIdx.x * blockDim.x + threadIdx.x) * 4; i4 < total;
             i4 += (int64_t)gridDim.x * blockDim.x * 4) {
            float4 v = *reinterpret_cast<float4*>(h + i4);
            int col = (int)(i4 % f);
            if (bias) {
                float4 bb = *reinterpret_cast<const float4*>(bias + col);
                v.x += bb.x;
                v.y += bb.y;
                v.z += bb.z;
                v.w += bb.w;
            }
            v.x = apply_act(v.x, act);
            v.y = apply_act(v.y, act);
            v.z = apply_act(v.z, act);
            v.w = apply_act(v.w, act);
            *reinterpret_cast<float4*>(h + i4) = v;
        }
    } else {
        for (int64_t i = (int64_t)blockIdx.x * blockDim.x + threadIdx.x; i < total; i += (int64_t)gridDim.x * blockDim.x) {
            float v = h[i] + (bias ? bias[i % f] : 0.f);
            h[i] = apply_act(v, act);
        }
    }
}

__global__ __launch_bounds__(WG) void bias_act_bf16_kernel(unsigned short* __restrict__ h, int64_t n, int f,
                                                           const float* __restrict__ bias, int act) {
    const int64_t total = n * (int64_t)f;
    if ((f & 7) == 0) {
        for (int64_t i8 = ((int64_t)blockIdx.x * blockDim.x + threadIdx.x) * 8; i8 < total;
             i8 += (int64_t)gridDim.x * blockDim.x * 8) {
            uint4 p = *reinterpret_cast<uint4*>(h + i8);
            unsigned int w[4] = {p.x, p.y, p.z, p.w};
            int col = (int)(i8 % f);
#pragma unroll
            for (int t = 0; t < 4; ++t) {
                float lo = __uint_as_float(w[t] << 16), hi = __uint_as_float(w[t] & 0xffff0000u);
                if (bias) {
                    lo += bias[col + 2 * t];
                    hi += bias[col + 2 * t + 1];
                }
                w[t] = pack_bf16x2(apply_act(lo, act), apply_act(hi, act));
            }
            *reinterpret_cast<uint4*>(h + i8) = make_uint4(w[0], w[1], w[2], w[3]);
        }
    } else {
        for (int64_t i = (int64_t)blockIdx.x * blockDim.x + threadIdx.x; i < total; i += (int64_t)gridDim.x * blockDim.x) {
            float v = bf16_bits_to_f32(h[i]) + (bias ? bias[i % f] : 0.f);
            h[i] = f32_to_bf16_bits(apply_act(v, act));
        }
    }
}

template <int VEC, int NV>
__device__ __forceinline__ void add_row_bf16(const unsigned short* __restrict__ row, int d, int lane, float (&r)[NV * VEC]) {
#pragma unroll
    for (int i = 0; i < NV; ++i) {
        int e = (i * 64 + lane) * VEC;
        if (e < d) {
            if constexpr (VEC == 4) {
                uint2 p = *reinterpret_cast<const uint2*>(row + e);
                r[i * 4 + 0] += __uint_as_float(p.x << 16);
                r[i * 4 + 1] += __uint_as_float(p.x & 0xffff0000u);
                r[i * 4 + 2] += __uint_as_float(p.y << 16);
                r[i * 4 + 3] += __uint_as_float(p.y & 0xffff0000u);
            } else {
                r[i] += bf16_bits_to_f32(row[e]);
            }
        }
    }
}

template <int VEC, int NV>
__global__ __launch_bounds__(WG) void ln_colsum_kernel(const float* __restrict__ z, int64_t n, int d, float eps,
                                                       const unsigned short* __restrict__ add_bf16,
                                                       const float* __restrict__ add_bias,
                                                       const int32_t* __restrict__ slot_map,
                                                       const float* __restrict__ delta_rows,
                                                       float* __restrict__ z_out,
                                                       float* __restrict__ partial ,
                                                       const int* __restrict__ vl = nullptr, int vl_bags = 0) {
    const int lane = threadIdx.x & 63;
    const int wave = threadIdx.x >> 6;
    int bid = blockIdx.x, gdim = gridDim.x;
    if (vl) {
        const int* __restrict__ dsc = vl + 4 * vl[4 * vl_bags + bid];
        const int64_t row0 = dsc[1];
        bid -= dsc[0];
        n = dsc[2];
        gdim = dsc[3];
        z += row0 * d;
        if (add_bf16) add_bf16 += row0 * d;
        if (slot_map) slot_map += row0;
        if (z_out) z_out += row0 * d;
    }
    float acc[NV * VEC];
#pragma unroll
    for (int i = 0; i < NV * VEC; ++i) acc[i] = 0.f;
    float bias_r[NV * VEC];
    if (add_bias) load_row<VEC, NV>(add_bias, d, lane, bias_r);
    const float inv_d = 1.0f / (float)d;
    const int64_t rstride = (int64_t)gdim * WAVES;
    float nz[NV * VEC];
    uint2 nb[NV];
    auto issue = [&](int64_t row) __attribute__((always_inline)) {
        load_row<VEC, NV>(z + row * d, d, lane, nz);
        if constexpr (VEC == 4) {
            if (add_bf16) {
#pragma unroll
                for (int i = 0; i < NV; ++i) {
                    const int e = (i * 64 + lane) * 4;
                    nb[i] = (e < d) ? *reinterpret_cast<const uint2*>(add_bf16 + row * d + e) : make_uint2(0u, 0u);
                }
            }
        }
    };
    int64_t row = (int64_t)bid * WAVES + wave;
    if (row < n) issue(row);
    for (; row < n; row += rstride) {
        float r[NV * VEC];
#pragma unroll
        for (int i = 0; i < NV * VEC; ++i) r[i] = nz[i];
        if constexpr (VEC == 4) {
            if (add_bf16) {
#pragma unroll
                for (int i = 0; i < NV; ++i) {
                    r[i * 4 + 0] += __uint_as_float(nb[i].x << 16);
                    r[i * 4 + 1] += __uint_as_float(nb[i].x & 0xffff0000u);
                    r[i * 4 + 2] += __uint_as_float(nb[i].y << 16);
                    r[i * 4 + 3] += __uint_as_float(nb[i].y & 0xffff0000u);
                }
            }
        } else {
            if (add_bf16) add_row_bf16<VEC, NV>(add_bf16 + row * d, d, lane, r);
        }
        if (row + rstride < n) issue(row + rstride);
        if (add_bias) {
#pragma unroll
            for (int i = 0; i < NV * VEC; ++i) r[i] += bias_r[i];
        }
        if (slot_map) {
            int sl = slot_map[row];
            if (sl >= 0) {
                float dr[NV * VEC];
                load_row<VEC, NV>(delta_rows + (int64_t)sl * d, d, lane, dr);
#pragma unroll
                for (int i = 0; i < NV * VEC; ++i) r[i] += dr[i];
            }
        }
        if (z_out) store_row_f32<VEC, NV>(z_out + row * d, d, lane, r);
        float s1 = 0.f;
#pragma unroll
        for (int i = 0; i < NV * VEC; ++i) s1 += r[i];
        const float mean = wave_sum(s1) * inv_d;
        float s2 = 0.f;
#pragma unroll
        for (int i = 0; i < NV; ++i) {
#pragma unroll
            for (int t = 0; t < VEC; ++t) {
                int e = (i * 64 + lane) * VEC + t;
                float dv = (e < d) ? (r[i * VEC + t] - mean) : 0.f;
                s2 = fmaf(dv, dv, s2);
            }
        }
        const float rstd = 1.0f / sqrtf(wave_sum(s2) * inv_d + eps);
#pragma unroll
        for (int i = 0; i < NV * VEC; ++i) acc[i] += (r[i] - mean) * rstd;
    }
    extern __shared__ float lds[];
    float* mine = lds + wave * (NV * VEC * 64);
#pragma unroll
    for (int i = 0; i < NV * VEC; ++i) mine[i * 64 + lane] = acc[i];
    __syncthreads();
    if (wave == 0) {
#pragma unroll
        for (int i = 0; i < NV; ++i) {
#pragma unroll
            for (int t = 0; t < VEC; ++t) {
                float s = 0.f;
                for (int w2 = 0; w2 < WAVES; ++w2) s += lds[w2 * (NV * VEC * 64) + (i * VEC + t) * 64 + lane];
                int e = (i * 64 + lane) * VEC + t;
                if (e < d) partial[(int64_t)blockIdx.x * d + e] = s;
            }
        }
    }
}

constexpr int HEAD_NSLICE = 16;
__global__ __launch_bounds__(256) void ln_colreduce_kernel(const float* __restrict__ partial, int nparts, int d,
                                                           float* __restrict__ partial2 ,
                                                           const int* __restrict__ vl = nullptr) {
    __shared__ float red[4][64];
    if (vl) {
        const int* __restrict__ dsc = vl + 4 * blockIdx.z;
        partial += (int64_t)dsc[0] * d;
        nparts = dsc[3];
        partial2 += (int64_t)blockIdx.z * HEAD_NSLICE * d;
    }
    const int c = threadIdx.x & 63, wv = threadIdx.x >> 6;
    const int e = blockIdx.x * 64 + c;
    const int sl = blockIdx.y;
    float s = 0.f;
    if (e < d)
        for (int p = sl + HEAD_NSLICE * wv; p < nparts; p += HEAD_NSLICE * 4) s += partial[(int64_t)p * d + e];
    red[wv][c] = s;
    __syncthreads();
    if (wv == 0 && e < d) partial2[(int64_t)sl * d + e] = ((red[0][c] + red[1][c]) + red[2][c]) + red[3][c];
}

__global__ __launch_bounds__(256) void head_gemv_kernel(const float* __restrict__ partial2, int64_t n, int d,
                                                        const float* __restrict__ gamma, const float* __restrict__ beta,
                                                        const float* __restrict__ w_head, const float* __restrict__ b_head,
                                                        float* __restrict__ pooled_out, float* __restrict__ logits,
                                                        const int* __restrict__ vl = nullptr) {
    __shared__ float red[256];
    if (vl) {
        partial2 += (int64_t)blockIdx.y * HEAD_NSLICE * d;
        n = vl[4 * blockIdx.y + 2];
        logits += (int64_t)blockIdx.y * gridDim.x;
// ... 627 lines not shown
        const int64_t total = n * (int64_t)d;
        if (aligned16(x) && aligned16(y)) {
            int64_t want = (total / 4 + WG - 1) / WG;
            int grid = (int)(want < (int64_t)snf::cu_count() * 8 ? (want > 0 ? want : 1) : (int64_t)snf::cu_count() * 8);
            hipLaunchKernelGGL(copy_f32_kernel, dim3(grid), dim3(WG), 0, s, x, y, total);
            int rc = snf::check_launch("copy_f32_kernel");
            if (rc) return rc;
        } else {
            if (hipMemcpyAsync(y, x, total * sizeof(float), hipMemcpyDeviceToDevice, s) != hipSuccess) {
                snf::set_error("snf_scatter_rows_f32: hipMemcpyAsync failed");
                return SNF_ELAUNCH;
            }
        }
    }
    if (k == 0) return SNF_OK;
    hipLaunchKernelGGL(scatter_rows_kernel<false>, dim3(k), dim3(WG), 0, s, y, n, d, idx, k, rows);
    return snf::check_launch("scatter_rows_kernel");
}

int snf_scatter_add_rows_f32(float* z, int64_t n, int d, const int64_t* idx, int k, const float* delta,
                             snf_stream_t stream) {
    SNF_REQUIRE(z && (k == 0 || (idx && delta)), "snf_scatter_add_rows_f32: null pointer");
    SNF_REQUIRE(n >= 1 && d >= 1 && k >= 0, "snf_scatter_add_rows_f32: bad shape");
    if (k == 0) return SNF_OK;
    hipLaunchKernelGGL(scatter_rows_kernel<true>, dim3(k), dim3(WG), 0, snf::as_stream(stream), z, n, d, idx, k, delta);
    return snf::check_launch("scatter_add_rows_kernel");
}

int snf_slot_map_i32(const int64_t* idx, int k, int64_t n, int32_t* map, snf_stream_t stream) {
    SNF_REQUIRE(map && (k == 0 || idx), "snf_slot_map_i32: null pointer");
    SNF_REQUIRE(n >= 1 && k >= 0, "snf_slot_map_i32: bad shape");
    hipStream_t s = snf::as_stream(stream);
    int64_t want = (n + 255) / 256;
    int grid = (int)(want < 2048 ? want : 2048);
    hipLaunchKernelGGL(fill_i32_kernel, dim3(grid), dim3(256), 0, s, map, n, -1);
    int rc = snf::check_launch("fill_i32_kernel");
    if (rc || k == 0) return rc;
    hipLaunchKernelGGL(slot_map_kernel, dim3((k + 255) / 256), dim3(256), 0, s, idx, k, n, map);
    return snf::check_launch("slot_map_kernel");
}

int snf_gather_slot_map_f32(const float* x, int64_t n, int d, const int64_t* idx, int k, float* xs, int32_t* map,
                            void* xs_bf16, snf_stream_t stream) {
    SNF_REQUIRE(x && map && (k == 0 || (idx && xs)), "snf_gather_slot_map_f32: null pointer");
    SNF_REQUIRE(n >= 1 && n < 0x7fffffffll && d >= 1 && k >= 0 && k <= 2048,
                "snf_gather_slot_map_f32: bad shape n=%lld d=%d k=%d (k <= 2048)", (long long)n, d, k);
    const int64_t grid = k + (n + WG - 1) / WG;
    hipLaunchKernelGGL(gather_slot_map_kernel, dim3((unsigned)grid), dim3(WG), 0, snf::as_stream(stream), x, n, d, idx, k, xs,
                       map, reinterpret_cast<__bf16*>(xs_bf16));
    return snf::check_launch("gather_slot_map_kernel");
}

int snf_bias_act(void* h, int dtype, int64_t n, int f, const float* bias, int act, snf_stream_t stream) {
    SNF_REQUIRE(h, "snf_bias_act: null h");
    SNF_REQUIRE(n >= 1 && f >= 1, "snf_bias_act: bad shape");
    SNF_REQUIRE(act >= SNF_ACT_RELU && act <= SNF_ACT_NONE, "snf_bias_act: unknown activation %d", act);
    SNF_REQUIRE(dtype == SNF_DT_F32 || dtype == SNF_DT_BF16, "snf_bias_act: unknown dtype %d", dtype);
    SNF_REQUIRE(aligned16(h) && (!bias || aligned16(bias)), "snf_bias_act: buffers must be 16-byte aligned");
    const int64_t total = n * (int64_t)f;
    const int per = dtype == SNF_DT_F32 ? 4 : 8;
    int64_t want = (total / per + WG - 1) / WG;
    int64_t cap = (int64_t)snf::cu_count() * 8;
    int grid = (int)(want < cap ? (want > 0 ? want : 1) : cap);
    hipStream_t s = snf::as_stream(stream);
    if (dtype == SNF_DT_F32)
        hipLaunchKernelGGL(bias_act_f32_kernel, dim3(grid), dim3(WG), 0, s, reinterpret_cast<float*>(h), n, f, bias, act);
    else
        hipLaunchKernelGGL(bias_act_bf16_kernel, dim3(grid), dim3(WG), 0, s, reinterpret_cast<unsigned short*>(h), n, f,
                           bias, act);
    return snf::check_launch("bias_act_kernel");
}

static int ln_head_parts(int64_t n) {
    int64_t want = (n + WAVES - 1) / WAVES;
    int64_t cap = (int64_t)snf::cu_count() * 4;
    return (int)(want < cap ? (want > 0 ? want : 1) : cap);
}

size_t snf_ln_mean_head_workspace_bytes(int d) {
    if (d < 1) return 0;
    return ((size_t)snf::cu_count() * 4 + HEAD_NSLICE) * (size_t)d * sizeof(float);
}

int snf_ln_mean_head_f32(const float* z, int64_t n, int d, const void* add_bf16, const float* add_bias,
                         const int32_t* slot_map, const float* delta_rows, float* z_out, const float* gamma,
                         const float* beta, float eps, const float* w_head, const float* b_head, int c_out, float* logits,
                         float* pooled, void* workspace, size_t workspace_bytes, snf_stream_t stream) {
    SNF_REQUIRE(z && w_head && logits && workspace, "snf_ln_mean_head_f32: null pointer");
    SNF_REQUIRE(!slot_map || delta_rows, "snf_ln_mean_head_f32: slot_map without delta_rows");
    SNF_REQUIRE(n >= 1 && d >= 1 && c_out >= 1, "snf_ln_mean_head_f32: bad shape");
    const int parts = ln_head_parts(n);
    if (workspace_bytes < ((size_t)parts + HEAD_NSLICE) * d * sizeof(float)) {
        snf::set_error("snf_ln_mean_head_f32: workspace %zu < %zu", workspace_bytes,
                       ((size_t)parts + HEAD_NSLICE) * d * sizeof(float));
        return SNF_EWORKSPACE;
    }
    RowCfg cfg;
    const bool al = aligned16(z) && (!add_bf16 || aligned16(add_bf16)) && (!add_bias || aligned16(add_bias)) &&
                    (!delta_rows || aligned16(delta_rows)) && (!z_out || aligned16(z_out));
    SNF_REQUIRE(pick_row_cfg(d, al, &cfg), "snf_ln_mean_head_f32: d=%d too wide (max 2048)", d);
    hipStream_t s = snf::as_stream(stream);
    float* partial = reinterpret_cast<float*>(workspace);
    float* partial2 = partial + (size_t)parts * d;
    SNF_ROW_DISPATCH(cfg, hipLaunchKernelGGL((ln_colsum_kernel<VEC, NV>), dim3(parts), dim3(WG),
                                              WAVES * NV * VEC * 64 * sizeof(float), s, z, n, d, eps,
                                              reinterpret_cast<const unsigned short*>(add_bf16), add_bias, slot_map,
                                              delta_rows, z_out, partial));
    int rc = snf::check_launch("ln_colsum_kernel");
    if (rc) return rc;
    hipLaunchKernelGGL(ln_colreduce_kernel, dim3((d + 63) / 64, HEAD_NSLICE), dim3(256), 0, s, partial, parts, d, partial2);
    rc = snf::check_launch("ln_colreduce_kernel");
    if (rc) return rc;
    hipLaunchKernelGGL(head_gemv_kernel, dim3(c_out), dim3(256), 0, s, partial2, n, d, gamma, beta, w_head, b_head, pooled,
                       logits);
    return snf::check_launch("head_gemv_kernel");
}

int snf_ln_mean_head_varlen_plan(const int64_t* offsets, int bags, int d, int32_t* table, size_t table_ints,
                                 size_t* table_ints_needed, size_t* workspace_bytes) {
    SNF_REQUIRE(offsets && bags >= 1 && d >= 1, "snf_ln_mean_head_varlen_plan: bad arguments");
    int64_t total = 0;
    for (int b = 0; b < bags; ++b) {
        const int64_t n = offsets[b + 1] - offsets[b];
        SNF_REQUIRE(n >= 1 && offsets[b + 1] < 0x7fffffffll, "snf_ln_mean_head_varlen_plan: bag %d has %lld rows", b, (long long)n);
        total += ln_head_parts(n);
    }
    SNF_REQUIRE(total < 0x3fffffff, "snf_ln_mean_head_varlen_plan: too many workgroups");
    const size_t need = (size_t)4 * bags + (size_t)total;
    if (table_ints_needed) *table_ints_needed = need;
    if (workspace_bytes) *workspace_bytes = ((size_t)total + (size_t)bags * HEAD_NSLICE) * d * sizeof(float);
    if (table) {
        SNF_REQUIRE(table_ints >= need, "snf_ln_mean_head_varlen_plan: table %zu < %zu ints", table_ints, need);
        int64_t wg = 0;
        for (int b = 0; b < bags; ++b) {
            const int64_t n = offsets[b + 1] - offsets[b];
            const int parts = ln_head_parts(n);
            table[4 * b + 0] = (int32_t)wg, table[4 * b + 1] = (int32_t)offsets[b], table[4 * b + 2] = (int32_t)n;
            table[4 * b + 3] = parts;
            for (int i = 0; i < parts; ++i) table[(size_t)4 * bags + wg + i] = b;
            wg += parts;
        }
    }
    return SNF_OK;
}

int snf_ln_mean_head_varlen_f32(const float* z, const int64_t* offsets, int bags, int d, const void* add_bf16,
                                const float* add_bias, const int32_t* slot_map, const float* delta_rows, float* z_out,
                                const float* gamma, const float* beta, float eps, const float* w_head, const float* b_head,
                                int c_out, float* logits, float* pooled, const int32_t* table_dev, void* workspace,
                                size_t workspace_bytes, snf_stream_t stream) {
    SNF_REQUIRE(z && offsets && w_head && logits && workspace && table_dev, "snf_ln_mean_head_varlen_f32: null pointer");
    SNF_REQUIRE(!slot_map || delta_rows, "snf_ln_mean_head_varlen_f32: slot_map without delta_rows");
    SNF_REQUIRE(bags >= 1 && d >= 1 && c_out >= 1, "snf_ln_mean_head_varlen_f32: bad shape");
    int64_t total = 0;
    for (int b = 0; b < bags; ++b) {
        SNF_REQUIRE(offsets[b + 1] > offsets[b], "snf_ln_mean_head_varlen_f32: empty bag %d", b);
        total += ln_head_parts(offsets[b + 1] - offsets[b]);
    }
    const size_t need = ((size_t)total + (size_t)bags * HEAD_NSLICE) * d * sizeof(float);
    if (workspace_bytes < need) {
        snf::set_error("snf_ln_mean_head_varlen_f32: workspace %zu < %zu", workspace_bytes, need);
        return SNF_EWORKSPACE;
    }
    RowCfg cfg;
    const bool al = aligned16(z) && (!add_bf16 || aligned16(add_bf16)) && (!add_bias || aligned16(add_bias)) &&
                    (!delta_rows || aligned16(delta_rows)) && (!z_out || aligned16(z_out));
    SNF_REQUIRE(pick_row_cfg(d, al, &cfg), "snf_ln_mean_head_varlen_f32: d=%d too wide (max 2048)", d);
    hipStream_t s = snf::as_stream(stream);
    float* partial = reinterpret_cast<float*>(workspace);
    float* partial2 = partial + (size_t)total * d;
    const int64_t n_all = offsets[bags];
    SNF_ROW_DISPATCH(cfg, hipLaunchKernelGGL((ln_colsum_kernel<VEC, NV>), dim3((unsigned)total), dim3(WG),
                                              WAVES * NV * VEC * 64 * sizeof(float), s, z, n_all, d, eps,
                                              reinterpret_cast<const unsigned short*>(add_bf16), add_bias, slot_map,
                                              delta_rows, z_out, partial, table_dev, bags));
    int rc = snf::check_launch("ln_colsum_kernel");
    if (rc) return rc;
    hipLaunchKernelGGL(ln_colreduce_kernel, dim3((d + 63) / 64, HEAD_NSLICE, bags), dim3(256), 0, s, partial, 0, d, partial2,
                       table_dev);
    rc = snf::check_launch("ln_colreduce_kernel");
    if (rc) return rc;
    hipLaunchKernelGGL(head_gemv_kernel, dim3(c_out, bags), dim3(256), 0, s, partial2, n_all, d, gamma, beta, w_head, b_head,
                       pooled, logits, table_dev);
    return snf::check_launch("head_gemv_kernel");
}

int snf_dropout_mask_f32(float dropout_p, uint64_t seed, uint64_t offset, int h, int64_t n, int k, float* mask,
                         snf_stream_t stream) {
    SNF_REQUIRE(mask && h >= 1 && n >= 1 && k >= 1, "snf_dropout_mask_f32: bad arguments");
    SNF_REQUIRE(dropout_p >= 0.f && dropout_p < 1.f, "snf_dropout_mask_f32: dropout_p=%f outside [0, 1)", dropout_p);
    const snf::DropoutState st = snf::make_dropout(dropout_p, seed, offset);
    const int64_t groups = (int64_t)h * n * ((k + 3) >> 2);
    hipLaunchKernelGGL(dropout_mask_kernel, dim3((unsigned)((groups + 255) / 256)), dim3(256), 0, snf::as_stream(stream), st, h, n, k,
                       mask, groups);
    return snf::check_launch("dropout_mask_kernel");
}

int snf_mil_loss_f32(const float* ins, int64_t n, int c, const float* logits, const float* label, const float* w, const float* pos_weight,
// ... 19 lines not shown
```

snuffy_amd/functional.py:

```python
import math

import torch
import torch.nn.functional as F

from . import ops
from ._ffi import SnuffyHipError

ACTIVATIONS = ("relu", "gelu", "leakyrelu", "selu")
FP32_ATTENTION = "x3"
X3_HL_ATTENTION = True
X3_HL_KPFRAG = True
X3_HL_KPFRAG_GATHER = True
FP32_GEMM = "x3"
BF16_DEEP_STACKS = "fp32"
FP32_SHARED_NORM = True
MFMA_ATTN_DK192 = False


def as_2d(x):
    if x.dim() == 3:
        if x.shape[0] != 1:
            raise IndexError("snuffy (binary) supports a single bag per forward: got batch %d" % x.shape[0])
        x = x[0]
    if x.dim() != 2:
# ... 130 lines not shown
        return offer[1]
    return None


def _take_xhat(layer, x2, eps):
    offer = getattr(layer, "_xhat_offer", None)
    layer._xhat_offer = None
    if offer is not None and offer[:4] == (x2.data_ptr(), tuple(x2.shape), x2._version, float(eps)):
        return offer[4]
    return None


def select_top(c1, big_lambda, top_share, n):
    k1 = min(math.ceil(big_lambda * top_share), n)
    if k1 < 1:
        return torch.empty(0, dtype=torch.int64, device=c1.device)
    return ops.topk(c1.detach(), k1)


def gather(x2, idx):
    return ops.gather_rows(x2, idx)


def layer_norm(x2, norm):
    if _needs_grad(x2, norm.weight, norm.bias):
        from . import autograd as SA
        return SA.LayerNormRowsFn.apply(x2, norm.weight, norm.bias, norm.eps)
    return ops.layernorm_rows(x2, norm.weight, norm.bias, norm.eps)


def act_name(ff):
    return ff.activation_name


def _drop_p(dropout):
    return float(dropout.p) if dropout is not None and getattr(dropout, "training", False) else 0.0


def attention_4d(query, key, value, dropout=None):
    b, h, n, dk = query.shape
    if b != 1:
        raise IndexError("single bag only")
    k = key.shape[2]
    q2 = query[0].transpose(0, 1).reshape(n, h * dk).contiguous()
    k2 = key[0].transpose(0, 1).reshape(k, h * dk).contiguous()
    v2 = value[0].transpose(0, 1).reshape(n, h * dk).contiguous()
    p_drop = _drop_p(dropout)
    if p_drop > 0.0 or _needs_grad(query, key, value):
        from . import autograd as SA
        out, attn = SA.SparseAttnFn.apply(q2, k2, v2, h, p_drop, False)
    else:
        out, attn, _ = ops.sparse_attn_fwd(q2, k2, v2, h, need_attn=True)
    return out.view(k, h, dk).transpose(0, 1).unsqueeze(0), attn.unsqueeze(0)


def mha_forward(mha, q_in, key_in, v_in, need_attn, precision):
    lq, lk, lv, lo = mha.linears
    q = F.linear(q_in, lq.weight, lq.bias)
    kp = F.linear(key_in, lk.weight, lk.bias)
    v = F.linear(v_in, lv.weight, lv.bias)
    p_drop = _drop_p(mha.dropout)
    if p_drop > 0.0 or _needs_grad(q, kp, v):
        from . import autograd as SA
        o, attn = SA.SparseAttnFn.apply(q, kp, v, mha.h, p_drop, False)
    else:
        o, attn, _ = ops.sparse_attn_fwd(q, kp, v, mha.h, need_attn=need_attn)
    out = F.linear(o, lo.weight, lo.bias)
    return out, (attn.unsqueeze(0) if attn is not None else None)


def ffn_forward(ff, x2, precision):
    p_drop = _drop_p(ff.dropout)
    if p_drop > 0.0 or _needs_grad(x2, ff.w_1.weight, ff.w_1.bias, ff.w_2.weight, ff.w_2.bias):
        from . import autograd as SA
        hid = SA._ACT[ff.activation_name](F.linear(x2, ff.w_1.weight, ff.w_1.bias))
        return F.linear(ff.dropout(hid), ff.w_2.weight, ff.w_2.bias)
    hid = torch.mm(x2, ff.w_1.weight.t())
    ops.bias_act_(hid, ff.w_1.bias, ff.activation_name)
    return F.linear(hid, ff.w_2.weight, ff.w_2.bias)


class Parts:

    __slots__ = ("base", "add_bf16", "add_bias", "slot", "delta")

    def __init__(self, base, add_bf16=None, add_bias=None, slot=None, delta=None):
        self.base, self.add_bf16, self.add_bias, self.slot, self.delta = base, add_bf16, add_bias, slot, delta

    @property
    def plain(self):
        return self.add_bf16 is None and self.add_bias is None and self.slot is None


_MATERIALIZE_CONST = {}


def materialize(parts):
    if parts.plain:
        return parts.base
    d = parts.base.shape[1]
    key = (parts.base.device, d)
    const = _MATERIALIZE_CONST.get(key)
    if const is None:
        const = (torch.zeros(1, d, dtype=torch.float32, device=parts.base.device),
                 torch.ones(d, dtype=torch.float32, device=parts.base.device))
        _MATERIALIZE_CONST[key] = const
    dummy_w, ones = const
    _, _, z = ops.ln_mean_head(parts.base, ones, dummy_w[0], 1e-5, dummy_w, None, parts.add_bf16, parts.add_bias,
                               parts.slot, parts.delta, want_z=True)
    return z


def head(parts, norm, linear, packed=None):
    if packed is not None:
        logits, _ = ops.ln_mean_head_varlen(parts.base, packed, norm.weight, norm.bias, norm.eps, linear.weight, linear.bias,
                                            parts.add_bf16, parts.add_bias, parts.slot, parts.delta)
        return logits
    if torch.is_grad_enabled() and (parts.base.requires_grad or norm.weight.requires_grad or linear.weight.requires_grad):
        from . import autograd as SA
        return SA.head_train(materialize(parts), norm, linear)
    logits, _, _ = ops.ln_mean_head(parts.base, norm.weight, norm.bias, norm.eps, linear.weight, linear.bias,
                                    parts.add_bf16, parts.add_bias, parts.slot, parts.delta)
    return logits


def _folded(layer, dkp=None):
    n0, n1 = layer.sublayer[0].norm, layer.sublayer[1].norm
    lq, lk, lv, lo = layer.self_attn.linears
    ff = layer.feed_forward
    plist = [n0.weight, n0.bias, n1.weight, n1.bias, lq.weight, lq.bias, lv.weight, lv.bias, ff.w_1.weight,
             ff.w_1.bias, ff.w_2.weight, lk.weight, lk.bias]
    hh = layer.self_attn.h
    dk0 = lq.weight.shape[0] // hh
    dkp = dk0 if dkp is None else dkp
    key = tuple(param_key(p) for p in plist) + (dkp,)
    ent = getattr(layer, "_fold", None)
    if ent is not None and ent[0] == key:
        return ent[1]
    if dkp != dk0:
        with torch.no_grad():
            bf = torch.bfloat16
            g0, b0, g1, b1 = (t.detach().float() for t in (n0.weight, n0.bias, n1.weight, n1.bias))
            wqv, bqv = _qv_weights(layer, dkp)
            w1 = ff.w_1.weight.detach().float()
            bqv_f = (wqv.float() @ b0 + bqv.float()).contiguous()
            b1f = (w1 @ b1 + ff.w_1.bias.detach().float()).contiguous()
            out = dict(wqv=(wqv.float() * g0).to(bf).contiguous(), bqv=bqv_f.to(bf), bqv_f=bqv_f,
                       w1=(w1 * g1).to(bf).contiguous(), b1=b1f, b1h=b1f.to(bf), w2=ff.w_2.weight.detach().to(bf),
                       wk=None, bk=None)
        layer._fold = (key, out)
        return out
    with torch.no_grad():
        g0, b0, g1, b1 = n0.weight, n0.bias, n1.weight, n1.bias
        d, f = lq.weight.shape[1], ff.w_1.weight.shape[0]
        bf = torch.bfloat16
        if lq.weight.is_cuda and d <= 2048 and lq.weight.dtype == torch.float32:
            dev = lq.weight.device
            wqv = torch.empty(2 * d, d, dtype=bf, device=dev)
            bqv_f = torch.empty(2 * d, dtype=torch.float32, device=dev)
            bqv = torch.empty(2 * d, dtype=bf, device=dev)
            ops.fold_linear(lq.weight, g0, b0, lq.bias, wqv[:d], bqv_f[:d], bqv[:d])
            ops.fold_linear(lv.weight, g0, b0, lv.bias, wqv[d:], bqv_f[d:], bqv[d:])
            w1 = torch.empty(f, d, dtype=bf, device=dev)
            b1f = torch.empty(f, dtype=torch.float32, device=dev)
            b1h = torch.empty(f, dtype=bf, device=dev)
            ops.fold_linear(ff.w_1.weight, g1, b1, ff.w_1.bias, w1, b1f, b1h)
            out = dict(wqv=wqv, bqv=bqv, bqv_f=bqv_f, w1=w1, b1=b1f, b1h=b1h, w2=ff.w_2.weight.to(bf),
                       wk=lk.weight.to(bf).contiguous(), bk=lk.bias.to(bf).contiguous())
        else:
            out = dict(
                wqv=torch.cat([lq.weight * g0, lv.weight * g0]).to(torch.bfloat16).contiguous(),
                bqv=torch.cat([lq.weight @ b0 + lq.bias, lv.weight @ b0 + lv.bias]).to(torch.bfloat16).contiguous(),
                bqv_f=torch.cat([lq.weight @ b0 + lq.bias, lv.weight @ b0 + lv.bias]).float().contiguous(),
                w1=(ff.w_1.weight * g1).to(torch.bfloat16), b1=(ff.w_1.weight @ b1 + ff.w_1.bias).contiguous(),
                b1h=(ff.w_1.weight @ b1 + ff.w_1.bias).to(torch.bfloat16),
                w2=ff.w_2.weight.to(torch.bfloat16),
                wk=lk.weight.to(torch.bfloat16).contiguous(), bk=lk.bias.to(torch.bfloat16).contiguous(),
            )
    layer._fold = (key, out)
    return out


def head_pad(dk):
    if dk in (64, 128):
        return dk
    if dk % 16 == 0 and 64 < dk < 128:
        return 128
    if dk % 16 == 0 and 16 <= dk < 64:
        return 64
    return None


def packed_head_pad(dk):
    if dk in (64, 128):
        return dk
    if dk % 16 == 0 and 64 < dk < 128:
        return 128
    return None


def _rows_linear_padded(x, w, bias, out_dtype=torch.float32):
    if x.shape[0] <= 8192:
        return ops.linear_rows_x3(x, w, bias, out_dtype=out_dtype)
    return torch.cat([ops.linear_rows_x3(x[i:i + 8192], w, bias, out_dtype=out_dtype) for i in range(0, x.shape[0], 8192)])

# ... 46 lines not shown
    ff = layer.feed_forward
    plist = [lq.weight, lq.bias, lv.weight, lv.bias, ff.w_1.weight, ff.w_1.bias, ff.w_2.weight, ff.w_2.bias]
    dkp = lq.weight.shape[0] // layer.self_attn.h if dkp is None else dkp
    key = tuple(param_key(p) for p in plist) + (dkp,)
    ent = getattr(layer, "_fold3", None)
    if ent is not None and ent[0] == key:
        return ent[1]
    with torch.no_grad():
        wqv, bqv = _qv_weights(layer, dkp)
        out = dict(
            wqv=ops.split3_weight(wqv),
            bqv=bqv.float().contiguous(),
            w1=ops.split3_weight(ff.w_1.weight), b1=ff.w_1.bias.detach().float().contiguous(),
            w2=ops.split3_weight(ff.w_2.weight), b2=ff.w_2.bias.detach().float().contiguous(),
        )
    out["_wqv_f32"] = wqv
    layer._fold3 = (key, out)
    return out


def _hl_weights(layer, fw):
    if "hl" not in fw:
        ff = layer.feed_forward
        with torch.no_grad():
            fw["hl"] = dict(wqv=ops.split_hl_weight(fw["_wqv_f32"]), w1=ops.split_hl_weight(ff.w_1.weight),
                            w2=ops.split_hl_weight(ff.w_2.weight))
    return fw["hl"]


def _hl_weights_folded(layer, dkp=None):
    n0, n1 = layer.sublayer[0].norm, layer.sublayer[1].norm
    lq, lk, lv, lo = layer.self_attn.linears
    ff = layer.feed_forward
    plist = [n0.weight, n0.bias, n1.weight, n1.bias, lq.weight, lq.bias, lv.weight, lv.bias, ff.w_1.weight, ff.w_1.bias]
    dkp = lq.weight.shape[0] // layer.self_attn.h if dkp is None else dkp
    key = tuple(param_key(p) for p in plist) + (dkp,)
    ent = getattr(layer, "_fold3f", None)
    if ent is not None and ent[0] == key:
        return ent[1]
    with torch.no_grad():
        g0, b0, g1, b1 = (t.double() for t in (n0.weight, n0.bias, n1.weight, n1.bias))
        wqv, bqv = (t.double() for t in _qv_weights(layer, dkp))
        w1, bb1 = ff.w_1.weight.double(), ff.w_1.bias.double()
        out = dict(wqv=ops.split_hl_weight((wqv * g0).float().contiguous()), bqv=(wqv @ b0 + bqv).float().contiguous(),
                   w1=ops.split_hl_weight((w1 * g1).float().contiguous()), b1=(w1 @ b1 + bb1).float().contiguous())
    layer._fold3f = (key, out)
    return out


_PARAM_CACHES = ("_snf_x3", "_snf_x3t", "_snf_img_hl", "_snf_img_cat")


def drop_param_caches(module):
    for prm in module.parameters():
        for name in _PARAM_CACHES:
            if hasattr(prm, name):
                delattr(prm, name)


def invalidate_folded(layer):
    layer._fold = None
    layer._fold3 = None
    layer._fold3f = None
    layer._fold3t = None
    layer._fold3t_hl = None
    layer._fold_pad = None
    layer._xhat_offer = None
    layer._xn3_offer = None
    drop_param_caches(layer)


def _rows_linear(x, lin):
    m, k = x.shape
    n = lin.weight.shape[0]
    if FP32_GEMM == "x3" and not _needs_grad(x, lin.weight, lin.bias) and x.dtype == torch.float32 and lin.weight.dtype == torch.float32:
        if m >= 2048 and ops.gemm_x3_supported(m, n, k):
            return ops.gemm_x3(ops.split3_rows(x), split3_cached(lin.weight), None if lin.bias is None else lin.bias.detach(),
                               out_dtype=torch.float32)
        if m < 2048 and ops.linear_rows_x3_supported(m, n, k):
            return ops.linear_rows_x3(x, lin.weight.detach(), None if lin.bias is None else lin.bias.detach())
    return F.linear(x, lin.weight, lin.bias)


def encoder_layer(x2, sel, layer, need_attn, precision, packed=None, ragged=None, last=False):
    if packed is None and torch.is_grad_enabled() and (x2.requires_grad or any(p.requires_grad for p in layer.parameters())):
        from . import autograd as SA
        return SA.encoder_layer_train(x2, sel, layer, need_attn, precision)
    n, d = x2.shape
    mha, ff = layer.self_attn, layer.feed_forward
    h = mha.h
    k = sel.shape[0]
    kb = k // packed.bags if packed is not None else k
    if ragged is not None:
        if packed is None or ragged.total != k or not ops.ragged_attn_supported(ragged.kmax, d // h):
            raise SnuffyHipError("ragged packed bags: %d keys (max %d per bag) at head width %d is outside the ragged attention "
                                 "kernel" % (k, ragged.kmax, d // h))
    elif packed is not None and (kb < 1 or not ops.varlen_attn_chunks_supported(precision, kb, packed_head_pad(d // h) or d // h)):
        raise SnuffyHipError("packed bags: %d keys per bag at head width %d is outside the varlen attention kernels" % (kb, d // h))
    n0, n1 = layer.sublayer[0].norm, layer.sublayer[1].norm
    lq, lk, lv, lo = mha.linears
    if k == 0:
        attn = torch.empty(1, h, n, 0, device=x2.device) if need_attn else None
        yn = ops.layernorm_rows(x2, n1.weight, n1.bias, n1.eps)
        hid = torch.mm(yn, ff.w_1.weight.t())
        ops.bias_act_(hid, ff.w_1.bias, ff.activation_name)
        z = torch.addmm(x2, hid, ff.w_2.weight.t())
        ops.bias_act_(z, ff.w_2.bias, "none")
        return Parts(z), attn

    if precision == "fp32" and FP32_GEMM == "x3" and ops.gemm_supported(n, d, 3 * ff.w_2.weight.shape[1]) \
            and ops.gemm_supported(n, 2 * d, 3 * d):
        f = ff.w_1.weight.shape[0]
        dk = d // h
        dkp = head_pad(dk) if (FP32_ATTENTION == "x3" and X3_HL_ATTENTION) else None
        hl_attn = (ragged is None and packed is None and dkp is not None and d % 16 == 0 and ops.x3_hl_attn_supported(k, dkp)
                   and lk.weight.dtype == torch.float32 and (dkp == dk or ops.gemm_supported(n, 2 * h * dkp, 3 * d)))
        if not hl_attn:
            dkp = dk
        if packed is not None and ragged is None and lk.weight.dtype == torch.float32 and d % 16 == 0:
            dkp = packed_head_pad(dk) or dk
        dp = h * dkp
        fw = _split_weights(layer, dkp)
        hl = d % 32 == 0 and f % 32 == 0 and ops.hl_eligible(n, 2 * dp, d) and ops.hl_eligible(n, f, d) and ops.hl_eligible(n, d, f)
        fh = _hl_weights(layer, fw) if hl else None
        shared = hl and shared_norm_layer(layer)
        fhf = _hl_weights_folded(layer, dkp) if shared else None
        xn3 = _take_xn3(layer, x2, n0, shared)
        fp = _padded_heads(layer, dkp) if dkp != dk else None
        wk, bk = (lk.weight.detach(), None if lk.bias is None else lk.bias.detach()) if fp is None else (fp["wk"], fp["bk"])
        scale = 1.0 / math.sqrt(dk)
        frag_ok = hl_attn and X3_HL_KPFRAG and ops.x3_hl_kpfrag_supported(k, h, dkp) and x2.dtype == torch.float32
        fused_gather = frag_ok and X3_HL_KPFRAG_GATHER and d % 16 == 0
        if fused_gather:
            kp, xs, slot = ops.gather_linear_rows_x3_kpfrag(x2, sel, wk, bk, h, scale=scale)
        else:
            xs, slot = ops.gather_slot_map(x2, sel)
        if fused_gather:
            pass
        elif frag_ok:
            kp = ops.linear_rows_x3_kpfrag(xs, wk, bk, h, scale=scale)
        elif fp is not None:
            kp = _rows_linear_padded(xs, wk, bk)
        else:
            kp = _rows_linear(xs, lk)
        if hl:
            if xn3 is None:
                xn3 = ops.layernorm_rows_hl(x2, None if shared else n0.weight, None if shared else n0.bias, n0.eps)
            if shared:
                qv = ops.gemm_hl(xn3, fhf["wqv"], fhf["bqv"], hl_out=hl_attn)
            else:
                qv = ops.gemm_hl(xn3, fh["wqv"], fw["bqv"], hl_out=hl_attn)
        else:
            xn3 = ops.layernorm_rows_split3(x2, n0.weight, n0.bias, n0.eps)
            qv = ops.gemm_x3(xn3, fw["wqv"], fw["bqv"], out_dtype=torch.float32, hl_out=hl_attn)
        if not shared:
            del xn3
        q, v = (None, None) if hl_attn else (qv[:, :dp], qv[:, dp:])
        if hl_attn:
            o, attn, _ = ops.sparse_attn_fwd_x3_hl(qv[:, :2 * dp], qv[:, 2 * dp:], kp, h, need_attn=need_attn,
                                                   scale=None if isinstance(kp, ops.KpFrag) else scale)
        elif ragged is not None:
            o, attn, _ = ops.sparse_attn_fwd_ragged(q, v, kp, packed, ragged, h, need_attn=need_attn)
        elif packed is not None:
            o, attn, _ = ops.sparse_attn_fwd_x3_varlen(q, v, kp, packed, kb, h, scale=scale, need_attn=need_attn)
        elif FP32_ATTENTION == "x3" and ops.x3_attn_supported(k, d // h):
            o, attn, _ = ops.sparse_attn_fwd_x3(q, v, kp, h, need_attn=need_attn)
        elif FP32_ATTENTION == "x3" and ops.x3u_attn_supported(k, d // h):
            o, attn, _ = ops.sparse_attn_fwd_x3u(q, kp, v, h, need_attn=need_attn)
        else:
            o, attn, _ = ops.sparse_attn_fwd(q.contiguous(), kp, v.contiguous(), h, need_attn=need_attn)
        del q, v, qv
        x_sel = None
        if fp is not None:
            delta = _rows_linear_padded(o, fp["wo"], None if lo.bias is None else lo.bias.detach())
        elif (not shared and FP32_GEMM == "x3" and lo.weight.dtype == torch.float32 and o.shape[0] < 2048
                and ops.linear_rows_x3_supported(o.shape[0], lo.weight.shape[0], o.shape[1])):
            delta, x_sel = ops.linear_rows_x3_resid(o, lo.weight.detach(), None if lo.bias is None else lo.bias.detach(), xs)
        else:
            delta = _rows_linear(o, lo)
        if shared:
            ops.layernorm_rows_hl_patch_(xn3, sel, xs, delta, eps=n1.eps)
            hid3 = ops.gemm_hl(xn3, fhf["w1"], fhf["b1"], ff.activation_name, hl_out=True)
            del xn3
            z = ops.gemm_hl(hid3, fh["w2"], fw["b2"], resid=x2)
        elif hl:
            if x_sel is None:
                x_sel = xs + delta
            yn3 = ops.layernorm_rows_hl(x2, n1.weight, n1.bias, n1.eps, slot=slot, patch_rows=x_sel)
            hid3 = ops.gemm_hl(yn3, fh["w1"], fw["b1"], ff.activation_name, hl_out=True)
            del yn3
            z = ops.gemm_hl(hid3, fh["w2"], fw["b2"], resid=x2)
        else:
            if x_sel is None:
                x_sel = xs + delta
            yn3 = ops.layernorm_rows_split3(x2, n1.weight, n1.bias, n1.eps, slot=slot, patch_rows=x_sel)
            hid3 = ops.gemm_x3(yn3, fw["w1"], fw["b1"], ff.activation_name, split3=True)
            del yn3
            z = ops.gemm_x3(hid3, fw["w2"], fw["b2"], out_dtype=torch.float32, resid=x2)
        del hid3
        if last:
            return Parts(z, slot=slot, delta=delta), (attn.unsqueeze(0) if attn is not None else None)
        ops.scatter_add_rows_(z, sel, delta)
        return Parts(z), (attn.unsqueeze(0) if attn is not None else None)

    if precision == "fp32":
        xs, slot = ops.gather_slot_map(x2, sel)
        kp = _rows_linear(xs, lk)
        xn = ops.layernorm_rows(x2, n0.weight, n0.bias, n0.eps)
        q = F.linear(xn, lq.weight, lq.bias)
        v = F.linear(xn, lv.weight, lv.bias)
        if ragged is not None:
            o, attn, _ = ops.sparse_attn_fwd_ragged(q, v, kp, packed, ragged, h, need_attn=need_attn)
        elif packed is not None:
            o, attn, _ = ops.sparse_attn_fwd_x3_varlen(q, v, kp, packed, kb, h, need_attn=need_attn)
        elif FP32_ATTENTION == "x3" and ops.x3_attn_supported(k, d // h):
            o, attn, _ = ops.sparse_attn_fwd_x3(q, v, kp, h, need_attn=need_attn)
        else:
            o, attn, _ = ops.sparse_attn_fwd(q, kp, v, h, need_attn=need_attn)
        del q, v, xn
        delta = _rows_linear(o, lo)
        x_sel = xs + delta
        yn = ops.layernorm_rows(x2, n1.weight, n1.bias, n1.eps, slot=slot, patch_rows=x_sel)
        hid = torch.mm(yn, ff.w_1.weight.t())
        del yn
        ops.bias_act_(hid, ff.w_1.bias, ff.activation_name)
        z = torch.addmm(x2, hid, ff.w_2.weight.t())
        del hid
        ops.bias_act_(z, ff.w_2.bias, "none")
        ops.scatter_add_rows_(z, sel, delta)
        return Parts(z), (attn.unsqueeze(0) if attn is not None else None)

    if n0.eps != n1.eps:
        raise NotImplementedError("bf16 path shares one normalisation between both sublayers: eps must match")
    dk = d // h
    dkp = head_pad(dk) if (ragged is None and packed is None and lk.weight.dtype == torch.float32) else dk
    if packed is not None and ragged is None and lk.weight.dtype == torch.float32 and d % 16 == 0:
        dkp = packed_head_pad(dk) or dk
        if dkp != dk and not ops.gemm_supported(n, 2 * h * dkp, d):
            dkp = dk
    elif dkp is None or (dkp != dk and not (ops.mfma_attn_supported(k, dkp, n, 2 * h * dkp) and ops.linear_rows_x3_supported(k, h * dkp, d)
                                         and ops.gemm_supported(n, 2 * h * dkp, d))):
        dkp = dk
    dp = h * dkp
    fw = _folded(layer, dkp)
    fp = _padded_heads(layer, dkp) if dkp != dk else None
    xhat = _take_xhat(layer, x2, n0.eps)
    if xhat is None:
        xhat = torch.empty(n, d, dtype=torch.bfloat16, device=x2.device)
        ops.layernorm_rows(x2, None, None, n0.eps, out=xhat)
    qv = ops.linear_bf16(xhat, fw["wqv"], fw["bqv_f"], fw["bqv"])
    q, v = qv[:, :dp], qv[:, dp:]
    dk192 = (MFMA_ATTN_DK192 and dkp == 192 and ragged is None and packed is None
             and ops.mfma_attn_dk192_supported(k, n, qv.stride(0)))
    if ragged is None and (packed is not None or dk192 or ops.mfma_attn_supported(k, dkp, n, qv.stride(0))):
        xs, slot, xs16 = ops.gather_slot_map(x2, sel, bf16_copy=True)
        if fp is not None:
            kp = _rows_linear_padded(xs, fp["wk"], fp["bk"], out_dtype=torch.bfloat16)
        elif (FP32_GEMM == "x3" and xs.shape[0] < 2048 and ops.linear_rows_x3_supported(xs.shape[0], d, d)
                and lk.weight.dtype == torch.float32):
            kp = ops.linear_rows_x3(xs, lk.weight.detach(), lk.bias.detach(), out_dtype=torch.bfloat16)
        else:
            kp = torch.addmm(fw["bk"], xs16, fw["wk"].t())
        if packed is not None:
            o, attn, _ = ops.sparse_attn_fwd_mfma_varlen(q, v, kp, packed, kb, h, scale=1.0 / math.sqrt(dk), need_attn=need_attn)
        else:
            o, attn, _ = ops.sparse_attn_fwd_mfma(q, v, kp, n, h, scale=1.0 / math.sqrt(dk), need_attn=need_attn)
    else:
        xs, slot = ops.gather_slot_map(x2, sel)
        kp = _rows_linear(xs, lk)
        if ragged is not None:
            qvf = qv.float()
            o, attn, _ = ops.sparse_attn_fwd_ragged(qvf[:, :d], qvf[:, d:], kp, packed, ragged, h, need_attn=need_attn)
            del qvf
        else:
            o, attn, _ = ops.sparse_attn_fwd(q.float(), kp, v.float(), h, need_attn=need_attn)
    del q, v, qv
    if fp is not None:
        delta = _rows_linear_padded(o, fp["wo"], None if lo.bias is None else lo.bias.detach())
    else:
        delta = _rows_linear(o, lo)
    x_sel = xs + delta
    ops.layernorm_rows(x_sel, None, None, n1.eps, out=xhat, out_row_idx=sel)
    hid = ops.linear_bf16(xhat, fw["w1"], fw["b1"], fw["b1h"], ff.activation_name)
    zb = ops.linear_bf16(hid, fw["w2"])
# ... 4 lines not shown
```

snuffy_amd/ops.py:

```python
import ctypes
import math

import torch

from . import _ffi
from ._ffi import ACT_CODES, DT_BF16, DT_BF16_HL, DT_BF16_SPLIT3, DT_F32, TOPK_MAX_K, check


def _p(t):
    return None if t is None else ctypes.c_void_p(t.data_ptr())


_raw_stream = getattr(torch._C, "_cuda_getCurrentRawStream", None)


def _stream():
    if _raw_stream is not None:
        return ctypes.c_void_p(_raw_stream(torch.cuda.current_device()))
    return ctypes.c_void_p(torch.cuda.current_stream().cuda_stream)


def _on_current_device(t, name):
    if t.device.index != torch.cuda.current_device():
        raise _ffi.SnuffyHipError("%s lives on %s but the current device is cuda:%d: select the tensor's device first "
# ... 324 lines not shown
    return dx, dxb, sums[0], sums[1]


def colsum_fused(src, row_weight=None, gate=None, want_bf16=False, inplace=False, dropout=None):
    if src.dtype not in (torch.float32, torch.bfloat16):
        raise TypeError("colsum_fused: src must be float32 or bfloat16")
    src = _req(src, src.dtype, "src", 2)
    n, d = src.shape
    if d % 8 or d > 8192:
        raise ValueError("colsum_fused: d=%d must be a multiple of 8 and <= 8192" % d)
    ws = 0
    if row_weight is not None:
        if row_weight.dtype != torch.float32 or not row_weight.is_cuda or row_weight.dim() != 1 or row_weight.shape[0] != n:
            raise ValueError("colsum_fused: row_weight must be a 1-D float32 GPU tensor of %d values (any stride)" % n)
        ws = row_weight.stride(0)
    if gate is not None:
        gate = _req(gate, torch.bfloat16, "gate", 2)
        if gate.shape != src.shape:
            raise ValueError("colsum_fused: gate shape %s does not match src %s" % (tuple(gate.shape), tuple(src.shape)))
    dst = None
    if inplace:
        if src.dtype != torch.bfloat16:
            raise TypeError("colsum_fused: inplace needs a bfloat16 src")
        dst = src
    elif want_bf16:
        dst = torch.empty(n, d, dtype=torch.bfloat16, device=src.device)
    lib = _ffi.load()
    part = torch.empty(lib.snf_colsum_blocks(n), d, dtype=torch.float32, device=src.device)
    if dropout is not None:
        if row_weight is not None or gate is not None:
            raise ValueError("colsum_fused: the dropout form takes no row weight and no gate")
        check(lib.snf_colsum_fused_dropout(_p(src), DT_F32 if src.dtype == torch.float32 else DT_BF16, n, d, float(dropout[0]),
                                           int(dropout[1]) & (2 ** 64 - 1), int(dropout[2]) & (2 ** 64 - 1), _p(dst), _p(part), _stream()),
              "snf_colsum_fused_dropout")
        return part.sum(0), dst
    check(lib.snf_colsum_fused(_p(src), DT_F32 if src.dtype == torch.float32 else DT_BF16, n, d, _p(row_weight), ws, _p(gate),
                               _p(dst), _p(part), _stream()), "snf_colsum_fused")
    return part.sum(0), dst


def fold_linear(w, gamma, beta, bias, out_w, out_bf=None, out_bf16=None):
    w = _req(w, torch.float32, "w", 2)
    r, c = w.shape
    gamma = _req(gamma, torch.float32, "gamma", 1)
    beta = _req(beta, torch.float32, "beta", 1)
    if bias is not None:
        bias = _req(bias, torch.float32, "bias", 1)
    if out_w.dtype != torch.bfloat16 or out_w.shape != (r, c) or out_w.stride(1) != 1:
        raise ValueError("fold_linear: out_w must be a [%d, %d] bfloat16 view with unit column stride" % (r, c))
    check(_ffi.load().snf_fold_linear_f32(_p(w), r, c, _p(gamma), _p(beta), _p(bias), _p(out_w), out_w.stride(0), _p(out_bf),
                                          _p(out_bf16), _stream()), "snf_fold_linear_f32")


def unfold_linear(dwf, w, gamma, beta, dbf):
    dwf = _req(dwf, torch.float32, "dwf", 2)
    w = _req(w, torch.float32, "w", 2)
    r, c = w.shape
    gamma = _req(gamma, torch.float32, "gamma", 1)
    beta = _req(beta, torch.float32, "beta", 1)
    dbf = _req(dbf, torch.float32, "dbf", 1)
    lib = _ffi.load()
    dw = torch.empty(r, c, dtype=torch.float32, device=w.device)
    part = torch.empty(lib.snf_fold_blocks(r), 2, c, dtype=torch.float32, device=w.device)
    check(lib.snf_unfold_linear_f32(_p(dwf), _p(w), r, c, _p(gamma), _p(beta), _p(dbf), _p(dw), _p(part), _stream()),
          "snf_unfold_linear_f32")
    sums = part.sum(0)
    return dw, sums[0], sums[1]


def bias_act_(h, bias, act):
    if not h.is_cuda or not h.is_contiguous() or h.dim() != 2:
        raise _ffi.SnuffyHipError("bias_act_: h must be a contiguous 2-D GPU tensor")
    dt = {torch.float32: DT_F32, torch.bfloat16: DT_BF16}.get(h.dtype)
    if dt is None:
        raise TypeError("bias_act_: h must be float32 or bfloat16")
    if bias is not None:
        bias = _req(bias, torch.float32, "bias", 1)
    check(_ffi.load().snf_bias_act(_p(h), dt, h.shape[0], h.shape[1], _p(bias), ACT_CODES[act], _stream()),
          "snf_bias_act")
    return h


def ln_mean_head(z, gamma, beta, eps, w_head, b_head, add_bf16=None, add_bias=None, slot=None, delta_rows=None,
                 want_z=False):
    z = _req(z, torch.float32, "z", 2)
    n, d = z.shape
    if add_bf16 is not None:
        add_bf16 = _req(add_bf16, torch.bfloat16, "add_bf16", 2)
    if add_bias is not None:
        add_bias = _req(add_bias, torch.float32, "add_bias", 1)
    if slot is not None:
        slot = _req(slot, torch.int32, "slot", 1)
        delta_rows = _req(delta_rows, torch.float32, "delta_rows", 2)
    z_out = torch.empty_like(z) if want_z else None
    gamma = _req(gamma, torch.float32, "gamma", 1)
    beta = _req(beta, torch.float32, "beta", 1)
    w_head = _req(w_head, torch.float32, "w_head", 2)
    if b_head is not None:
        b_head = _req(b_head, torch.float32, "b_head", 1)
    c = w_head.shape[0]
    lib = _ffi.load()
    logits = torch.empty(c, dtype=torch.float32, device=z.device)
    pooled = torch.empty(d, dtype=torch.float32, device=z.device)
    wsb = lib.snf_ln_mean_head_workspace_bytes(d)
    ws = _ws(wsb, z.device)
    check(lib.snf_ln_mean_head_f32(_p(z), n, d, _p(add_bf16), _p(add_bias), _p(slot), _p(delta_rows), _p(z_out),
                                   _p(gamma), _p(beta), float(eps), _p(w_head), _p(b_head), c, _p(logits), _p(pooled),
                                   _p(ws), wsb, _stream()), "snf_ln_mean_head_f32")
    return logits, pooled, z_out


def attn_bwd_dropout_supported(k, dk):
    return 1 <= k <= 1024 and k % 4 == 0 and dk % 8 == 0


def sparse_attn_bwd(q, kp, v, p, dout, h, mask=None, scale=None, dropout=None):
    if q.dtype != torch.float32 or v.dtype != torch.float32:
        raise TypeError("sparse_attn_bwd: q and v must be float32")
    kp = _req(kp, torch.float32, "kp", 2)
    if q.dim() == 2 and kp.dim() == 2 and (q.shape[1] // h) % 8 == 0 and kp.shape[0] <= 1024:
        q, v = _rows16(q, "q"), _rows16(v, "v")
    else:
        q, v = _req(q, torch.float32, "q", 2), _req(v, torch.float32, "v", 2)
    p = _req(p, torch.float32, "p", 3)
    dout = _req(dout, torch.float32, "dout", 2)
    if mask is not None:
        mask = _req(mask, torch.float32, "mask", 3)
    n, d = q.shape
    k = kp.shape[0]
    dk = d // h
    if p.shape != (h, n, k) or dout.shape != (k, d) or (mask is not None and mask.shape != p.shape):
        raise ValueError("sparse_attn_bwd: inconsistent shapes")
    scale = 1.0 / math.sqrt(dk) if scale is None else scale
    lib = _ffi.load()
    dq = torch.empty(n, d, dtype=torch.float32, device=q.device)
    dv = torch.empty(n, d, dtype=torch.float32, device=q.device)
    dkp = torch.empty_like(kp)
    wsb = lib.snf_sparse_attn_bwd_workspace_bytes(n, k, h, dk)
    ws = _ws(wsb, q.device)
    if dropout is not None and mask is None and float(dropout[0]) > 0.0:
        check(lib.snf_sparse_attn_bwd_dropout_f32(_p(q), q.stride(0), _p(kp), _p(v), v.stride(0), _p(p), float(dropout[0]),
                                                  int(dropout[1]) & (2 ** 64 - 1), int(dropout[2]) & (2 ** 64 - 1), _p(dout), n, k, h, dk,
                                                  float(scale), _p(dq), _p(dkp), _p(dv), _p(ws), wsb, _stream()),
              "snf_sparse_attn_bwd_dropout_f32")
        return dq, dkp, dv
    check(lib.snf_sparse_attn_bwd_ld_f32(_p(q), q.stride(0), _p(kp), _p(v), v.stride(0), _p(p), _p(mask), _p(dout), n, k, h, dk, float(scale),
                                         _p(dq), _p(dkp), _p(dv), _p(ws), wsb, _stream()), "snf_sparse_attn_bwd_ld_f32")
    return dq, dkp, dv


def mfma_attn_bwd_supported(k, dk):
    return (dk == 128 and 1 <= k <= 224) or (dk == 64 and 1 <= k <= 256)


def mfma_attn_train_chunks_supported(k, dk):
    return (dk == 128 and 1 <= k <= 8 * 224) or (dk == 64 and 1 <= k <= 8 * 256)


def sparse_attn_bwd_mfma(q, v, kp, dout, lse, h, mask=None, scale=None, dropout=None, fused_bf16_grads=False):
    if q.dtype not in (torch.float32, torch.bfloat16) or v.dtype != q.dtype:
        raise TypeError("sparse_attn_bwd_mfma: q and v must both be float32 or both bfloat16")
    q = _rows16(q, "q")
    v = _rows16(v, "v")
    kp = _req(kp, torch.float32, "kp", 2)
    dout = _req(dout, torch.float32, "dout", 2)
    lse = _req(lse, torch.float32, "lse", 2)
    if mask is not None:
        mask = _req(mask, torch.float32, "mask", 3)
    n, d = q.shape
    k = kp.shape[0]
    dk = d // h
    scale = 1.0 / math.sqrt(dk) if scale is None else scale
    lib = _ffi.load()
    if fused_bf16_grads:
        dqv = torch.empty(n, 2 * d, dtype=torch.bfloat16, device=q.device)
        dq, dv, ldd, gdt = dqv[:, :d], dqv[:, d:], 2 * d, DT_BF16
    else:
        dq = torch.empty(n, d, dtype=torch.float32, device=q.device)
        dv = torch.empty(n, d, dtype=torch.float32, device=q.device)
        ldd, gdt = d, DT_F32
    bf16 = q.dtype == torch.bfloat16
    ds = torch.empty(h, n, k, dtype=torch.bfloat16 if bf16 else torch.float32, device=q.device)
    dt = DT_F32 if q.dtype == torch.float32 else DT_BF16
    pdrop, seed, offset = dropout if dropout is not None else (0.0, 0, 0)
    if dk != 192 and (mfma_attn_bwd_supported(k, dk) or not mfma_attn_train_chunks_supported(k, dk)):
        check(lib.snf_sparse_attn_bwd_mfma_ex(_p(q), q.stride(0), _p(v), v.stride(0), dt, _p(kp), _p(dout), _p(lse), _p(mask),
                                              float(pdrop), int(seed) & (2 ** 64 - 1), int(offset) & (2 ** 64 - 1), n, k, h, dk,
                                              float(scale), _p(dq), _p(dv), ldd, gdt, _p(ds), DT_BF16 if bf16 else DT_F32, _stream()),
# ... 842 lines not shown
            out = torch.empty(m, 2 * n, dtype=torch.bfloat16, device=a_hl.device)
        odt = DT_BF16_HL
    else:
        if out is None:
            out = torch.empty(m, n, dtype=out_dtype, device=a_hl.device)
        odt = DT_F32 if out.dtype == torch.float32 else DT_BF16
    ldr = 0
    if resid is not None:
        if hl_out or out.dtype != torch.float32 or resid.dtype != torch.float32 or tuple(resid.shape) != (m, n):
            raise ValueError("gemm_hl: resid needs an fp32 [m, n] tensor and an fp32 output")
        resid = _rows16(resid, "resid")
        ldr = resid.stride(0)
    lib = _ffi.load()
    ws, ws_bytes = None, 0
    if GEMM_HL_SPLITK:
        ws_bytes = int(lib.snf_gemm_hl_ws_bytes(m, n, k2 // 2))
        if ws_bytes:
            ws = _hl_workspace(a_hl.device, ws_bytes)
    check(lib.snf_gemm_hl_ws_bf16(_p(a_hl), a_hl.stride(0), _p(w_hl), w_hl.stride(0), _p(bias), _p(resid), ldr, m, n, k2 // 2,
                                  ACT_CODES[act], _p(out), out.stride(0), odt, _p(ws), ws_bytes, _stream()), "snf_gemm_hl_ws_bf16")
    return out


def encoder_dropout_supported(n, d, f):
    return d % 32 == 0 and f % 32 == 0 and d <= 8192 and hl_eligible(n, f, d) and hl_eligible(n, d, f)


def gemm_hl_dropout(a_hl, w_hl, bias, dropout, act="none", hl_out=False, resid=None, out=None):
    if a_hl.dtype != torch.bfloat16 or w_hl.dtype != torch.bfloat16:
        raise TypeError("gemm_hl_dropout: operands must be bfloat16 hl images")
    if (act, bool(hl_out)) not in (("relu", True), ("none", False)):
        raise ValueError("gemm_hl_dropout: only relu -> hl image and none -> fp32 (+ resid) exist")
    a_hl = _rows16(a_hl, "a_hl")
    w_hl = _rows16(w_hl, "w_hl")
    m, k2 = a_hl.shape
    n = w_hl.shape[0]
    if w_hl.shape[1] != k2 or k2 % 64 or (hl_out and n % 32):
        raise ValueError("gemm_hl_dropout: images are %s and %s" % (tuple(a_hl.shape), tuple(w_hl.shape)))
    if bias is not None:
        bias = _req(bias, torch.float32, "bias", 1)
    if out is None:
        out = torch.empty(m, 2 * n, dtype=torch.bfloat16, device=a_hl.device) if hl_out else \
            torch.empty(m, n, dtype=torch.float32, device=a_hl.device)
    odt = DT_BF16_HL if hl_out else DT_F32
    ldr = 0
    if resid is not None:
        if hl_out or resid.dtype != torch.float32 or tuple(resid.shape) != (m, n):
            raise ValueError("gemm_hl_dropout: resid needs an fp32 [m, n] tensor and an fp32 output")
        resid = _rows16(resid, "resid")
        ldr = resid.stride(0)
    p, seed, offset = dropout
    lib = _ffi.load()
    ws, ws_bytes = None, 0
    if GEMM_HL_SPLITK:
        ws_bytes = int(lib.snf_gemm_hl_ws_bytes(m, n, k2 // 2))
        if ws_bytes:
            ws = _hl_workspace(a_hl.device, ws_bytes)
    check(lib.snf_gemm_hl_ws_dropout_bf16(_p(a_hl), a_hl.stride(0), _p(w_hl), w_hl.stride(0), _p(bias), _p(resid), ldr, m, n, k2 // 2,
                                          ACT_CODES[act], _p(out), out.stride(0), odt, float(p), int(seed) & (2 ** 64 - 1),
                                          int(offset) & (2 ** 64 - 1), _p(ws), ws_bytes, _stream()), "snf_gemm_hl_ws_dropout_bf16")
    return out


def gemm_hl_gated(a_hl, w_hl, gate_hl):
    a_hl, w_hl, gate_hl = _rows16(a_hl, "a_hl"), _rows16(w_hl, "w_hl"), _rows16(gate_hl, "gate_hl")
    if a_hl.dtype != torch.bfloat16 or w_hl.dtype != torch.bfloat16 or gate_hl.dtype != torch.bfloat16:
        raise TypeError("gemm_hl_gated: operands must be bfloat16 hl images")
    m, k2 = a_hl.shape
    n = w_hl.shape[0]
    if w_hl.shape[1] != k2 or k2 % 64 or n % 32 or tuple(gate_hl.shape) != (m, 2 * n):
        raise ValueError("gemm_hl_gated: inconsistent shapes")
    out = torch.empty(m, 2 * n, dtype=torch.bfloat16, device=a_hl.device)
    check(_ffi.load().snf_gemm_hl_gated_bf16(_p(a_hl), a_hl.stride(0), _p(w_hl), w_hl.stride(0), _p(gate_hl), gate_hl.stride(0), m, n,
                                             k2 // 2, _p(out), out.stride(0), _stream()), "snf_gemm_hl_gated_bf16")
    return out


def hl_colsum(img):
    s, _ = colsum_fused(img)
    return s.view(-1, 2, 32).sum(1).reshape(-1)


GEMM_HL_SPLITK = True


def _hl_workspace(device, nbytes):
    return _ws(nbytes, device)


def split3_weight(w, colscale=None):
    w = w.detach().float()
    if colscale is not None:
        colscale = colscale.detach().float().contiguous()
    if w.is_cuda and w.dim() == 2 and w.shape[1] % 8 == 0 and w.stride(1) == 1 and w.stride(0) % 4 == 0 and w.data_ptr() % 16 == 0:
        out = torch.empty(w.shape[0], 3 * w.shape[1], dtype=torch.bfloat16, device=w.device)
        check(_ffi.load().snf_split3_weight_f32(_p(w), w.stride(0), w.shape[0], w.shape[1], _p(colscale), _p(out), _stream()),
              "snf_split3_weight_f32")
        return out
    if colscale is not None:
        w = w * colscale
    hi = w.to(torch.bfloat16)
    lo = (w - hi.float()).to(torch.bfloat16)
    return torch.cat([hi, lo, hi], dim=1).contiguous()


def split3_rows(x):
    if x.dtype != torch.float32:
        raise TypeError("split3_rows: x must be float32")
    x = _rows16(x, "x")
    m, k = x.shape
    if k % 8:
        hi = x.to(torch.bfloat16)
        lo = (x - hi.float()).to(torch.bfloat16)
        return torch.cat([hi, hi, lo], dim=1).contiguous()
    out = torch.empty(m, 3 * k, dtype=torch.bfloat16, device=x.device)
    check(_ffi.load().snf_split3_f32(_p(x), x.stride(0), m, k, _p(out), _stream()), "snf_split3_f32")
    return out


def split3_colsum(x, gate=None, out=None, col=0, want_colsum=True):
    if x.dtype != torch.float32:
        raise TypeError("split3_colsum: x must be float32")
    x = _rows16(x, "x")
    m, k = x.shape
    if k % 8 or k > 8192:
        raise ValueError("split3_colsum: k=%d must be a multiple of 8 and <= 8192" % k)
    ldg = 0
    if gate is not None:
        if gate.dtype != torch.bfloat16 or tuple(gate.shape) != (m, k):
            raise ValueError("split3_colsum: gate must be bfloat16 of the shape of x")
        gate = _rows16(gate, "gate")
        ldg = gate.stride(0)
    if out is None:
        out = torch.empty(m, 3 * k, dtype=torch.bfloat16, device=x.device)
        col = 0
    elif (out.dtype != torch.bfloat16 or out.dim() != 2 or not out.is_contiguous() or out.shape[0] != m or out.shape[1] % 3
          or col % 8 or col + k > out.shape[1] // 3):
        raise ValueError("split3_colsum: bad out image")
    plane = out.shape[1] // 3
    lib = _ffi.load()
    part = torch.empty(lib.snf_colsum_blocks(m), k, dtype=torch.float32, device=x.device) if want_colsum else None
    dst = out if col == 0 else out[:, col:]
    check(lib.snf_split3_colsum_f32(_p(x), x.stride(0), m, k, _p(gate), ldg, _p(dst), out.stride(0), plane, _p(part), _stream()),
          "snf_split3_colsum_f32")
    return out, (part.sum(0) if part is not None else None)


def split_hl_colsum(x, gate_hl=None, out=None, col=0, want_colsum=True, dropout=None):
    if x.dtype != torch.float32:
        raise TypeError("split_hl_colsum: x must be float32")
    x = _rows16(x, "x")
    m, k = x.shape
    if k % 32 or k > 8192:
        raise ValueError("split_hl_colsum: k=%d must be a multiple of 32 and <= 8192" % k)
    ldg = 0
    if gate_hl is not None:
        if gate_hl.dtype != torch.bfloat16 or tuple(gate_hl.shape) != (m, 2 * k):
            raise ValueError("split_hl_colsum: gate must be the bfloat16 hl image of a matrix of the shape of x")
        gate_hl = _rows16(gate_hl, "gate")
        ldg = gate_hl.stride(0)
    if out is None:
        out = torch.empty(m, 2 * k, dtype=torch.bfloat16, device=x.device)
        col = 0
    elif (out.dtype != torch.bfloat16 or out.dim() != 2 or not out.is_contiguous() or out.shape[0] != m or out.shape[1] % 64
          or col % 32 or 2 * (col + k) > out.shape[1]):
        raise ValueError("split_hl_colsum: bad out image")
# ... 153 lines not shown
```

snuffy_amd/snuffy.py:

```python
import copy
import math

import numpy as np
import torch
import torch.nn as nn

from . import functional as SF
from . import ops

device = torch.device("cuda" if torch.cuda.is_available() else "cpu")


class RuntimeConfig:

    def __init__(self, precision="fp32", return_attention=True):
        self.stack = None
        self.sampler = "reference"
        self._device_sampler = None
        self._draws = 0
        self.set(precision, return_attention)

    def set_sampler(self, sampler):
        if sampler not in ("reference", "device"):
            raise ValueError("sampler must be 'reference' or 'device', got %r" % (sampler,))
# ... 187 lines not shown


class MultiHeadedAttention(nn.Module):

    def __init__(self, h, d_model, dropout=0.1):
        super(MultiHeadedAttention, self).__init__()
        assert d_model % h == 0
        self.d_big_lambda = d_model // h
        self.h = h
        self.linears = clones(nn.Linear(d_model, d_model), 4)
        self.attn = None
        self.dropout = nn.Dropout(p=dropout)
        self.cfg = RuntimeConfig()

    def forward(self, query, key, value):
        out, self.attn = SF.mha_forward(self, SF.as_2d(query), SF.as_2d(key), SF.as_2d(value), True,
                                        self.cfg.precision)
        return out.unsqueeze(0), self.attn


class PositionwiseFeedForward(nn.Module):

    def __init__(self, d_model, d_ff, activation, dropout=0.1):
        super(PositionwiseFeedForward, self).__init__()
        self.w_1 = nn.Linear(d_model, d_ff)
        self.w_2 = nn.Linear(d_ff, d_model)
        self.dropout = nn.Dropout(dropout)
        if activation not in SF.ACTIVATIONS:
            raise KeyError(activation)
        self.activation_name = activation
        self.cfg = RuntimeConfig()

    def forward(self, x):
        return SF.ffn_forward(self, SF.as_2d(x), self.cfg.precision).view(x.shape)


class MILNet(nn.Module):

    def __init__(self, i_classifier, b_classifier):
        super(MILNet, self).__init__()
        self.i_classifier = i_classifier
        self.b_classifier = b_classifier

    def configure(self, precision=None, return_attention=None, graph_max_patches=None, sampler=None):
        self.b_classifier.configure(precision, return_attention)
        if sampler is not None:
            self.b_classifier.cfg.set_sampler(sampler)
        if graph_max_patches is not None:
            self._graph_max_patches = int(graph_max_patches)
            self._graphs, self._graph_seen, self._graph_pool = {}, set(), None
        return self

    def forward(self, x):
        if self._graph_ok(x):
            return self._forward_graph(x)
        return self._forward_eager(x)

    def _forward_eager(self, x):
        for layer in self.b_classifier.encoder.layers[:1]:
            layer._xhat_offer = None
            layer._xn3_offer = None
        feats, classes = self._critic(x)
        prediction_bag, A = self.b_classifier(feats, classes)
        return classes, prediction_bag, A

    _GRAPH_SHAPES = 1024
    _GRAPH_COPY_BYTES = 32 << 20

    def _graph_ok(self, x):
        lim = getattr(self, "_graph_max_patches", 0)
        if lim <= 0 or self.training or torch.is_grad_enabled():
            return False
        if not (isinstance(x, torch.Tensor) and x.is_cuda and x.dim() == 3 and x.shape[0] == 1 and x.dtype == torch.float32
                and x.is_contiguous() and 0 < x.shape[1] <= lim and type(self.i_classifier) is FCLayer):
            return False
        if self.b_classifier.cfg.return_attention and x.numel() * 4 > self._GRAPH_COPY_BYTES:
            return False
        on_device = self.b_classifier.cfg.sampler == "device"
        return all(type(l) is EncoderLayer and (l.random_patch_share == 0 or on_device) for l in self.b_classifier.encoder.layers)

    def _weights_signature(self):
        plist = list(self.parameters())
        knobs = tuple((l.big_lambda, l.random_patch_share) for l in self.b_classifier.encoder.layers)
        knobs += (SF.FP32_GEMM, SF.FP32_ATTENTION, SF.X3_HL_ATTENTION, SF.X3_HL_KPFRAG, SF.X3_HL_KPFRAG_GATHER, SF.FP32_SHARED_NORM, ops.GEMM_HL_SPLITK,
                  SF.BF16_DEEP_STACKS, self.b_classifier.cfg.sampler)
        return tuple(SF.param_key(p) for p in plist), knobs

    def invalidate(self):
        if getattr(self, "_graph_max_patches", 0):
            self._graphs.clear()
            self._graph_seen.clear()
            self._graph_sig = None
        for layer in self.b_classifier.encoder.layers:
            SF.invalidate_folded(layer)
        SF.drop_param_caches(self)
        return self

    _GRAPH_STATE = ("_graphs", "_graph_seen", "_graph_pool", "_graph_sig", "_packed_bags", "_capture_stream")

    def __deepcopy__(self, memo):
        new = self.__class__.__new__(self.__class__)
        memo[id(self)] = new
        for k, v in self.__dict__.items():
            if k not in self._GRAPH_STATE:
                new.__dict__[k] = copy.deepcopy(v, memo)
        if getattr(self, "_graph_max_patches", 0):
            new._graphs, new._graph_seen, new._graph_pool = {}, set(), None
        new.b_classifier.cfg._device_sampler = None
        return new

    def _forward_graph(self, x):
        sig = self._weights_signature()
        if sig != getattr(self, "_graph_sig", None):
            self._graphs.clear()
            self._graph_seen.clear()
            self._graph_sig = sig
        cfg = self.b_classifier.cfg
        small = x.numel() * 4 <= self._GRAPH_COPY_BYTES
        key = (tuple(x.shape), x.device, cfg.precision, cfg.return_attention) + (() if small else (x.data_ptr(),))
        ent = self._graphs.get(key)
        if ent is None:
            if not small and key not in self._graph_seen:
                if len(self._graph_seen) > 8192:
                    self._graph_seen.clear()
                self._graph_seen.add(key)
                return self._forward_eager(x)
            try:
                static_x = torch.empty_like(x).copy_(x) if small else x
                cur = torch.cuda.current_stream()
                side = getattr(self, "_capture_stream", None)
                if side is None or side.device != x.device:
                    side = self._capture_stream = torch.cuda.Stream(x.device)
                side.wait_stream(cur)
                with torch.cuda.stream(side):
                    sel_state = ops.fresh_selector(x.device)
                    for _ in range(2):
                        self._forward_eager(static_x)
                cur.wait_stream(side)
                if self._graph_pool is None:
                    self._graph_pool = torch.cuda.graph_pool_handle()
                graph = torch.cuda.CUDAGraph()
                graph._snf_selector = sel_state
                with torch.cuda.graph(graph, pool=self._graph_pool, stream=side, capture_error_mode="thread_local"):
                    out = self._forward_eager(static_x)
            except Exception as exc:
                import warnings
                warnings.warn("snuffy_amd: HIP-graph capture of the inference forward failed (%s: %s); graph replay is "
                              "disabled for this model, every kernel is issued from Python" % (type(exc).__name__, exc),
                              RuntimeWarning, stacklevel=2)
                self._graph_max_patches = 0
                torch.cuda.synchronize()
                return self._forward_eager(x)
            if len(self._graphs) >= self._GRAPH_SHAPES:
                self._graphs.pop(next(iter(self._graphs)))
            ent = self._graphs[key] = (graph, static_x, out)
        graph, static_x, out = ent
        if small:
            static_x.copy_(x)
        graph.replay()
        return tuple(o.clone() if isinstance(o, torch.Tensor) else o for o in out)

    def forward_bags(self, bags):
        from . import packed
        return packed.forward_bags(self, bags)

    def forward_packed(self, x_cat, packed_bags, ragged=False):
        from . import packed
# ... 44 lines not shown
```

Measured before the change: 886.7 slides/s.

## Defer split-K partial reduction of last FFN GEMM into LN-mean-head kernel

Adds a deferred split-K mode to the hl GEMM for the last encoder layer's FFN output projection. Split-K partial tiles stay in workspace slabs with a tile map instead of being reduced with tickets inside the GEMM. The layernorm/mean/head kernel then adds those slabs while it reads z. This removes the in-GEMM cross-workgroup reduction and its synchronization, at the cost of a second GEMM launch, extra slab reads in the LN kernel, and more register pressure there.

```diff
diff --git a/include/snuffy_hip.h b/include/snuffy_hip.h
--- a/include/snuffy_hip.h
+++ b/include/snuffy_hip.h
@@ -109,6 +109,11 @@
                          const int32_t* slot_map, const float* delta_rows, float* z_out, const float* gamma,
                          const float* beta, float eps, const float* w_head, const float* b_head, int c_out,
                          float* logits, float* pooled, void* workspace, size_t workspace_bytes, snf_stream_t stream);
+int snf_ln_mean_head_deferred_f32(const float* z, int64_t n, int d, const float* slabs, const int32_t* tile_map, int tiles_n,
+                                  const void* add_bf16, const float* add_bias, const int32_t* slot_map, const float* delta_rows,
+                                  float* z_out, const float* gamma, const float* beta, float eps, const float* w_head,
+                                  const float* b_head, int c_out, float* logits, float* pooled, void* workspace,
+                                  size_t workspace_bytes, snf_stream_t stream);
 
 size_t snf_sparse_attn_fwd_workspace_bytes(int64_t n, int k, int h, int dk, int mfma);
 int snf_sparse_attn_fwd_f32(const float* q, const float* kp, const float* v, int64_t n, int k, int h, int dk,
@@ -204,6 +209,10 @@
 int snf_gemm_hl_ws_bf16(const void* a_hl, int64_t lda, const void* w_hl, int64_t ldw, const float* bias, const float* resid,
                         int64_t ldr, int64_t m, int n, int k, int act, void* c, int64_t ldc, int out_dtype, void* workspace,
                         size_t workspace_bytes, snf_stream_t stream);
+size_t snf_gemm_hl_deferred_ws_bytes(int64_t m, int n, int k, size_t* slab_offset);
+int snf_gemm_hl_deferred_f32(const void* a_hl, int64_t lda, const void* w_hl, int64_t ldw, const float* bias, const float* resid,
+                             int64_t ldr, int64_t m, int n, int k, int act, float* c, int64_t ldc, int out_dtype, void* workspace,
+                             size_t workspace_bytes, snf_stream_t stream);
 int snf_gemm_hl_dropout_bf16(const void* a_hl, int64_t lda, const void* w_hl, int64_t ldw, const float* bias, const float* resid,
                              int64_t ldr, int64_t m, int n, int k, int act, void* c, int64_t ldc, int out_dtype, float dropout_p,
                              uint64_t seed, uint64_t offset, snf_stream_t stream);
diff --git a/snuffy_amd/_ffi.py b/snuffy_amd/_ffi.py
--- a/snuffy_amd/_ffi.py
+++ b/snuffy_amd/_ffi.py
@@ -68,6 +68,9 @@
     "snf_ln_mean_head_f32": (c_int, [c_void_p, c_int64, c_int, c_void_p, c_void_p, c_void_p, c_void_p, c_void_p,
                                      c_void_p, c_void_p, c_float, c_void_p, c_void_p, c_int, c_void_p, c_void_p,
                                      c_void_p, c_size_t, c_void_p]),
+    "snf_ln_mean_head_deferred_f32": (c_int, [c_void_p, c_int64, c_int, c_void_p, c_void_p, c_int, c_void_p, c_void_p, c_void_p, c_void_p,
+                                              c_void_p, c_void_p, c_void_p, c_float, c_void_p, c_void_p, c_int, c_void_p, c_void_p,
+                                              c_void_p, c_size_t, c_void_p]),
     "snf_sparse_attn_fwd_workspace_bytes": (c_size_t, [c_int64, c_int, c_int, c_int, c_int]),
     "snf_sparse_attn_fwd_f32": (c_int, [c_void_p, c_void_p, c_void_p, c_int64, c_int, c_int, c_int, c_float, c_void_p,
                                         c_void_p, c_void_p, c_void_p, c_size_t, c_void_p]),
@@ -144,6 +147,9 @@
     "snf_split_hl_colsum_f32": (c_int, [c_void_p, c_int64, c_int64, c_int, c_void_p, c_int64, c_void_p, c_int64, c_void_p, c_void_p]),
     "snf_gemm_hl_ws_bf16": (c_int, [c_void_p, c_int64, c_void_p, c_int64, c_void_p, c_void_p, c_int64, c_int64, c_int, c_int, c_int,
                                     c_void_p, c_int64, c_int, c_void_p, c_size_t, c_void_p]),
+    "snf_gemm_hl_deferred_ws_bytes": (c_size_t, [c_int64, c_int, c_int, c_void_p]),
+    "snf_gemm_hl_deferred_f32": (c_int, [c_void_p, c_int64, c_void_p, c_int64, c_void_p, c_void_p, c_int64, c_int64, c_int, c_int, c_int,
+                                         c_void_p, c_int64, c_int, c_void_p, c_size_t, c_void_p]),
     "snf_gemm_bf16_dropout": (c_int, [c_void_p, c_int64, c_void_p, c_int64, c_void_p, c_int64, c_int, c_int, c_int, c_void_p, c_int64,
                                       c_int, c_int, c_float, c_uint64, c_uint64, c_void_p]),
     "snf_dropout_rows_bf16": (c_int, [c_void_p, c_int64, c_int64, c_int, c_float, c_uint64, c_uint64, c_void_p]),
diff --git a/snuffy_amd/csrc/gemm.hip b/snuffy_amd/csrc/gemm.hip
--- a/snuffy_amd/csrc/gemm.hip
+++ b/snuffy_amd/csrc/gemm.hip
@@ -480,8 +480,10 @@
     if (wid < 4) __builtin_amdgcn_s_barrier();
 }
 
-template <int ACT, int OUT, bool SPLIT = false, bool GATE = false, bool DROP = false>
+template <int ACT, int OUT, int SPLIT_MODE = 0, bool GATE = false, bool DROP = false>
 __global__ __launch_bounds__(512, 2) void gemm_hl_kernel(GemmParams P) {
+    constexpr bool SPLIT = SPLIT_MODE != 0, DEFER = SPLIT_MODE == 2;
+    static_assert(!DEFER || (SPLIT && OUT == 1 && ACT == SNF_ACT_NONE && !GATE && !DROP), "gemm_hl: the deferred split writes plain fp32");
     static_assert(!GATE || (OUT == 3 && ACT == SNF_ACT_NONE && !SPLIT), "gemm_hl: the gated form writes an hl image, no activation, no split");
     static_assert(!DROP || (!GATE && (OUT == 1 || OUT == 3)), "gemm_hl: dropout goes with the fp32 and the hl-image outputs");
     constexpr int NI = 4, BN = 256;
@@ -783,7 +785,23 @@
             __builtin_amdgcn_s_setprio(0);
             buf ^= 1;
         }
-        if constexpr (SPLIT) {
+        int etile = tile;
+        bool efull = full;
+#ifdef SNF_GEMM_SPLIT_NOSUM
+        if constexpr (false) {
+#else
+        if constexpr (DEFER) {
+            if (sp_part != 0) {
+                int mark = sp_slot + 1;
+                asm volatile("" : "+s"(mark));
+                if (threadIdx.x == 0) reinterpret_cast<int*>(P.split_cnt)[tile] = mark;
+                P.c = P.split_slab + (size_t)sp_slot * (size_t)(BM * BN);
+                P.ldc = BN;
+                P.bias = nullptr, P.resid = nullptr;
+                etile = 0, efull = true;
+            }
+        } else if constexpr (SPLIT) {
+#endif
             volatile unsigned int& s_ticket = *reinterpret_cast<volatile unsigned int*>(smem);
             float* slab0 = P.split_slab + (size_t)sp_slot * P.split_cap * (size_t)(BM * BN);
             unsigned tix = threadIdx.x;
@@ -822,13 +840,13 @@
                     acc[mi][ni] = sum;
                 }
         }
-        load_bias(tile);
+        load_bias(etile);
         wait_vmcnt<0>();
         bias_landed();
-        if (full)
-            epilogue(tile, std::true_type{});
+        if (efull)
+            epilogue(etile, std::true_type{});
         else
-            epilogue(tile, std::false_type{});
+            epilogue(etile, std::false_type{});
         after_epilogue = true;
         if (!has_next) break;
         tile = next;
@@ -1339,6 +1357,91 @@
     return gemm_hl_ws_impl(a_hl, lda, w_hl, ldw, bias, resid, ldr, m, n, k, act, c, ldc, out_dtype, nullptr, workspace, workspace_bytes, stream);
 }
 
+namespace {
+struct HlDeferred {
+    HlSplit g;
+    int map_rcap;
+    size_t slab_offset, bytes;
+};
+HlDeferred hl_deferred_geometry(int64_t m, int n, int k) {
+    HlDeferred d = {hl_split_geometry(m, n, k), 0, 0, 0};
+    if (d.g.cap < 2) return d;
+    d.g.cap = 2;
+    const int ntiles = (int)(((m + BM - 1) / BM) * ((n + 255) / 256));
+    d.map_rcap = (ntiles + 7) / 8 > d.g.rcap ? (ntiles + 7) / 8 : d.g.rcap;
+    d.slab_offset = ((size_t)8 * d.map_rcap * sizeof(int32_t) + 4095) & ~(size_t)4095;
+    d.bytes = d.slab_offset + (size_t)8 * d.g.rcap * (size_t)(BM * 256) * sizeof(float);
+    return d;
+}
+
+int launch_hl_deferred(GemmParams P, const HlDeferred& d, hipStream_t s) {
+    constexpr int lds = 2 * 2 * BM * 128 + 8 * 4096;
+    auto kern = gemm_hl_kernel<SNF_ACT_NONE, 1>;
+    auto kern2 = gemm_hl_kernel<SNF_ACT_NONE, 1, 2>;
+    static thread_local unsigned long long attr_set_mask = 0, attr_set2_mask = 0;
+    if (int rc = snf::lds_opt_in(reinterpret_cast<const void*>(kern), lds, &attr_set_mask, "gemm_hl")) return rc;
+    if (int rc = snf::lds_opt_in(reinterpret_cast<const void*>(kern2), lds, &attr_set2_mask, "gemm_hl")) return rc;
+    const int ntiles = P.tiles_m * P.tiles_n;
+    int grid = snf::cu_count() & ~7;
+    if (grid < 8) grid = 8;
+    const int per_xcd = (ntiles + 7) / 8;
+    if (per_xcd * 8 < grid) grid = per_xcd * 8;
+    P.split_cap = 2, P.split_rcap = d.map_rcap;
+    hipLaunchKernelGGL(kern, dim3(grid), dim3(512), lds, s, P);
+    if (int rc = snf::check_launch("gemm_hl_kernel")) return rc;
+    P.split_rcap = d.g.rcap;
+    hipLaunchKernelGGL(kern2, dim3(grid), dim3(512), lds, s, P);
+    return snf::check_launch("gemm_hl_kernel<deferred split>");
+}
+}
+
+extern "C" size_t snf_gemm_hl_deferred_ws_bytes(int64_t m, int n, int k, size_t* slab_offset) {
+    const HlDeferred d = hl_deferred_geometry(m, n, k);
+    if (slab_offset) *slab_offset = d.slab_offset;
+    return d.bytes;
+}
+
+extern "C" int snf_gemm_hl_deferred_f32(const void* a_hl, int64_t lda, const void* w_hl, int64_t ldw, const float* bias, const float* resid,
+                                        int64_t ldr, int64_t m, int n, int k, int act, float* c, int64_t ldc, int out_dtype, void* workspace,
+                                        size_t workspace_bytes, snf_stream_t stream) {
+    SNF_REQUIRE(a_hl && w_hl && c && workspace, "snf_gemm_hl_deferred_f32: null pointer");
+    SNF_REQUIRE(m >= 1 && n >= 1 && k >= 1, "snf_gemm_hl_deferred_f32: bad shape m=%lld n=%d k=%d", (long long)m, n, k);
+    if (act != SNF_ACT_NONE || out_dtype != SNF_DT_F32) {
+        snf::set_error("snf_gemm_hl_deferred_f32: fp32 output without activation only (act %d, out_dtype %d)", act, out_dtype);
+        return SNF_EUNSUPPORTED;
+    }
+    SNF_REQUIRE(!resid || (ldr >= n && ldr % 4 == 0 && reinterpret_cast<uintptr_t>(resid) % 16 == 0),
+                "snf_gemm_hl_deferred_f32: a residual needs 16-byte aligned rows (ldr=%lld)", (long long)ldr);
+    const HlDeferred d = hl_deferred_geometry(m, n, k);
+    if (k % BKS || k < BKS || n % 8 || lda % 8 || ldw % 8 || ldc % 4 || lda < 2 * (int64_t)k || ldw < 2 * (int64_t)k || ldc < n ||
+        (reinterpret_cast<uintptr_t>(a_hl) | reinterpret_cast<uintptr_t>(w_hl) | reinterpret_cast<uintptr_t>(c)) % 16 ||
+        (bias && reinterpret_cast<uintptr_t>(bias) % 16) || m * lda >= 0x7fffffffll || (int64_t)n * ldw >= 0x7fffffffll || !d.bytes) {
+        snf::set_error("snf_gemm_hl_deferred_f32: shape m=%lld n=%d k=%d (lda %lld ldw %lld ldc %lld) outside the kernel's domain "
+                       "(snf_gemm_hl_bf16's, and a last round that splits: snf_gemm_hl_deferred_ws_bytes > 0)",
+                       (long long)m, n, k, (long long)lda, (long long)ldw, (long long)ldc);
+        return SNF_EUNSUPPORTED;
+    }
+    if (workspace_bytes < d.bytes || reinterpret_cast<uintptr_t>(workspace) % 128) {
+        snf::set_error("snf_gemm_hl_deferred_f32: workspace %zu < %zu (or not 128-byte aligned)", workspace_bytes, d.bytes);
+        return SNF_EWORKSPACE;
+    }
+    GemmParams P;
+    P.a = reinterpret_cast<const unsigned short*>(a_hl);
+    P.w = reinterpret_cast<const unsigned short*>(w_hl);
+    P.bias = bias;
+    P.c = c;
+    P.lda = lda, P.ldw = ldw, P.ldc = ldc;
+    P.m = (int)m, P.n = n, P.k = k, P.act = act;
+    P.tiles_m = (int)((m + BM - 1) / BM);
+    P.tiles_n = (n + 255) / 256;
+    P.trace = nullptr;
+    P.resid = resid;
+    P.ldr = ldr;
+    P.split_cnt = reinterpret_cast<unsigned int*>(workspace);
+    P.split_slab = reinterpret_cast<float*>(reinterpret_cast<unsigned char*>(workspace) + d.slab_offset);
+    return launch_hl_deferred(P, d, snf::as_stream(stream));
+}
+
 extern "C" int snf_gemm_hl_ws_dropout_bf16(const void* a_hl, int64_t lda, const void* w_hl, int64_t ldw, const float* bias,
                                            const float* resid, int64_t ldr, int64_t m, int n, int k, int act, void* c, int64_t ldc,
                                            int out_dtype, float dropout_p, uint64_t seed, uint64_t offset, void* workspace,
diff --git a/snuffy_amd/csrc/rowops.hip b/snuffy_amd/csrc/rowops.hip
--- a/snuffy_amd/csrc/rowops.hip
+++ b/snuffy_amd/csrc/rowops.hip
@@ -1073,7 +1073,7 @@
     }
 }
 
-template <int VEC, int NV>
+template <int VEC, int NV, bool DEFER = false>
 __global__ __launch_bounds__(WG) void ln_colsum_kernel(const float* __restrict__ z, int64_t n, int d, float eps,
                                                        const unsigned short* __restrict__ add_bf16,
                                                        const float* __restrict__ add_bias,
@@ -1081,7 +1081,9 @@
                                                        const float* __restrict__ delta_rows,
                                                        float* __restrict__ z_out,
                                                        float* __restrict__ partial ,
-                                                       const int* __restrict__ vl = nullptr, int vl_bags = 0) {
+                                                       const int* __restrict__ vl = nullptr, int vl_bags = 0,
+                                                       const float* __restrict__ slabs = nullptr,
+                                                       const int32_t* __restrict__ tile_map = nullptr, int tiles_n = 0) {
     const int lane = threadIdx.x & 63;
     const int wave = threadIdx.x >> 6;
     int bid = blockIdx.x, gdim = gridDim.x;
@@ -1105,8 +1107,36 @@
     const int64_t rstride = (int64_t)gdim * WAVES;
     float nz[NV * VEC];
     uint2 nb[NV];
+    constexpr int NCB = DEFER ? (NV * VEC * 64 + 255) / 256 : 1;
+    float ns[DEFER ? NV * VEC : 1];
+    int mp_n[NCB], mp_nn[NCB];
+    auto lookup = [&](int64_t row, int (&mp)[NCB]) __attribute__((always_inline)) {
+        const int trow = __builtin_amdgcn_readfirstlane((int)(row >> 8));
+#pragma unroll
+        for (int cb = 0; cb < NCB; ++cb) mp[cb] = cb < tiles_n ? tile_map[(int64_t)trow * tiles_n + cb] : 0;
+    };
     auto issue = [&](int64_t row) __attribute__((always_inline)) {
         load_row<VEC, NV>(z + row * d, d, lane, nz);
+        if constexpr (DEFER) {
+#pragma unroll
+            for (int i = 0; i < NV; ++i) {
+                const int sl = mp_n[i * 64 * VEC / 256];
+#pragma unroll
+                for (int t = 0; t < VEC; ++t) ns[i * VEC + t] = 0.f;
+                if (sl) {
+                    const int e = (i * 64 + lane) * VEC;
+                    const float* __restrict__ sp = slabs + ((int64_t)(sl - 1) * 256 + (row & 255)) * 256 + (e & 255);
+                    if constexpr (VEC == 4) {
+                        if (e < d) {
+                            const float4 t4 = *reinterpret_cast<const float4*>(sp);
+                            ns[i * 4 + 0] = t4.x, ns[i * 4 + 1] = t4.y, ns[i * 4 + 2] = t4.z, ns[i * 4 + 3] = t4.w;
+                        }
+                    } else {
+                        if (e < d) ns[i] = *sp;
+                    }
+                }
+            }
+        }
         if constexpr (VEC == 4) {
             if (add_bf16) {
 #pragma unroll
@@ -1118,11 +1148,28 @@
         }
     };
     int64_t row = (int64_t)bid * WAVES + wave;
+    if constexpr (DEFER) {
+        if (row < n) lookup(row, mp_n);
+    }
     if (row < n) issue(row);
+    if constexpr (DEFER) {
+        if (row + rstride < n) lookup(row + rstride, mp_nn);
+    }
     for (; row < n; row += rstride) {
         float r[NV * VEC];
 #pragma unroll
         for (int i = 0; i < NV * VEC; ++i) r[i] = nz[i];
+        if constexpr (DEFER) {
+#pragma unroll
+            for (int i = 0; i < NV; ++i) {
+                if (mp_n[i * 64 * VEC / 256]) {
+#pragma unroll
+                    for (int t = 0; t < VEC; ++t) r[i * VEC + t] += ns[i * VEC + t];
+                }
+            }
+#pragma unroll
+            for (int cb = 0; cb < NCB; ++cb) mp_n[cb] = mp_nn[cb];
+        }
         if constexpr (VEC == 4) {
             if (add_bf16) {
 #pragma unroll
@@ -1137,6 +1184,9 @@
             if (add_bf16) add_row_bf16<VEC, NV>(add_bf16 + row * d, d, lane, r);
         }
         if (row + rstride < n) issue(row + rstride);
+        if constexpr (DEFER) {
+            if (row + 2 * rstride < n) lookup(row + 2 * rstride, mp_nn);
+        }
         if (add_bias) {
 #pragma unroll
             for (int i = 0; i < NV * VEC; ++i) r[i] += bias_r[i];
@@ -1930,10 +1980,11 @@
     return ((size_t)snf::cu_count() * 4 + HEAD_NSLICE) * (size_t)d * sizeof(float);
 }
 
-int snf_ln_mean_head_f32(const float* z, int64_t n, int d, const void* add_bf16, const float* add_bias,
-                         const int32_t* slot_map, const float* delta_rows, float* z_out, const float* gamma,
-                         const float* beta, float eps, const float* w_head, const float* b_head, int c_out, float* logits,
-                         float* pooled, void* workspace, size_t workspace_bytes, snf_stream_t stream) {
+static int ln_mean_head_impl(const float* z, int64_t n, int d, const float* slabs, const int32_t* tile_map, int tiles_n,
+                             const void* add_bf16, const float* add_bias, const int32_t* slot_map, const float* delta_rows,
+                             float* z_out, const float* gamma, const float* beta, float eps, const float* w_head,
+                             const float* b_head, int c_out, float* logits, float* pooled, void* workspace, size_t workspace_bytes,
+                             snf_stream_t stream) {
     SNF_REQUIRE(z && w_head && logits && workspace, "snf_ln_mean_head_f32: null pointer");
     SNF_REQUIRE(!slot_map || delta_rows, "snf_ln_mean_head_f32: slot_map without delta_rows");
     SNF_REQUIRE(n >= 1 && d >= 1 && c_out >= 1, "snf_ln_mean_head_f32: bad shape");
@@ -1950,10 +2001,17 @@
     hipStream_t s = snf::as_stream(stream);
     float* partial = reinterpret_cast<float*>(workspace);
     float* partial2 = partial + (size_t)parts * d;
-    SNF_ROW_DISPATCH(cfg, hipLaunchKernelGGL((ln_colsum_kernel<VEC, NV>), dim3(parts), dim3(WG),
-                                              WAVES * NV * VEC * 64 * sizeof(float), s, z, n, d, eps,
-                                              reinterpret_cast<const unsigned short*>(add_bf16), add_bias, slot_map,
-                                              delta_rows, z_out, partial));
+    if (tile_map) {
+        SNF_ROW_DISPATCH(cfg, hipLaunchKernelGGL((ln_colsum_kernel<VEC, NV, true>), dim3(parts), dim3(WG),
+                                                  WAVES * NV * VEC * 64 * sizeof(float), s, z, n, d, eps,
+                                                  reinterpret_cast<const unsigned short*>(add_bf16), add_bias, slot_map,
+                                                  delta_rows, z_out, partial, nullptr, 0, slabs, tile_map, tiles_n));
+    } else {
+        SNF_ROW_DISPATCH(cfg, hipLaunchKernelGGL((ln_colsum_kernel<VEC, NV>), dim3(parts), dim3(WG),
+                                                  WAVES * NV * VEC * 64 * sizeof(float), s, z, n, d, eps,
+                                                  reinterpret_cast<const unsigned short*>(add_bf16), add_bias, slot_map,
+                                                  delta_rows, z_out, partial));
+    }
     int rc = snf::check_launch("ln_colsum_kernel");
     if (rc) return rc;
     hipLaunchKernelGGL(ln_colreduce_kernel, dim3((d + 63) / 64, HEAD_NSLICE), dim3(256), 0, s, partial, parts, d, partial2);
@@ -1962,6 +2020,26 @@
     hipLaunchKernelGGL(head_gemv_kernel, dim3(c_out), dim3(256), 0, s, partial2, n, d, gamma, beta, w_head, b_head, pooled,
                        logits);
     return snf::check_launch("head_gemv_kernel");
+}
+
+int snf_ln_mean_head_f32(const float* z, int64_t n, int d, const void* add_bf16, const float* add_bias,
+                         const int32_t* slot_map, const float* delta_rows, float* z_out, const float* gamma,
+                         const float* beta, float eps, const float* w_head, const float* b_head, int c_out, float* logits,
+                         float* pooled, void* workspace, size_t workspace_bytes, snf_stream_t stream) {
+    return ln_mean_head_impl(z, n, d, nullptr, nullptr, 0, add_bf16, add_bias, slot_map, delta_rows, z_out, gamma, beta, eps, w_head,
+                             b_head, c_out, logits, pooled, workspace, workspace_bytes, stream);
+}
+
+int snf_ln_mean_head_deferred_f32(const float* z, int64_t n, int d, const float* slabs, const int32_t* tile_map, int tiles_n,
+                                  const void* add_bf16, const float* add_bias, const int32_t* slot_map, const float* delta_rows,
+                                  float* z_out, const float* gamma, const float* beta, float eps, const float* w_head,
+                                  const float* b_head, int c_out, float* logits, float* pooled, void* workspace,
+                                  size_t workspace_bytes, snf_stream_t stream) {
+    SNF_REQUIRE(slabs && tile_map, "snf_ln_mean_head_deferred_f32: null slabs / tile map");
+    SNF_REQUIRE(aligned16(slabs) && tiles_n >= 1 && d <= 256 * (int64_t)tiles_n,
+                "snf_ln_mean_head_deferred_f32: d=%d beyond %d column tiles (or unaligned slabs)", d, tiles_n);
+    return ln_mean_head_impl(z, n, d, slabs, tile_map, tiles_n, add_bf16, add_bias, slot_map, delta_rows, z_out, gamma, beta, eps,
+                             w_head, b_head, c_out, logits, pooled, workspace, workspace_bytes, stream);
 }
 
 int snf_ln_mean_head_varlen_plan(const int64_t* offsets, int bags, int d, int32_t* table, size_t table_ints,
diff --git a/snuffy_amd/functional.py b/snuffy_amd/functional.py
--- a/snuffy_amd/functional.py
+++ b/snuffy_amd/functional.py
@@ -236,14 +236,15 @@
 
 class Parts:
 
-    __slots__ = ("base", "add_bf16", "add_bias", "slot", "delta")
-
-    def __init__(self, base, add_bf16=None, add_bias=None, slot=None, delta=None):
+    __slots__ = ("base", "add_bf16", "add_bias", "slot", "delta", "deferred")
+
+    def __init__(self, base, add_bf16=None, add_bias=None, slot=None, delta=None, deferred=None):
         self.base, self.add_bf16, self.add_bias, self.slot, self.delta = base, add_bf16, add_bias, slot, delta
+        self.deferred = deferred
 
     @property
     def plain(self):
-        return self.add_bf16 is None and self.add_bias is None and self.slot is None
+        return self.add_bf16 is None and self.add_bias is None and self.slot is None and self.deferred is None
 
 
 _MATERIALIZE_CONST = {}
@@ -261,12 +262,14 @@
         _MATERIALIZE_CONST[key] = const
     dummy_w, ones = const
     _, _, z = ops.ln_mean_head(parts.base, ones, dummy_w[0], 1e-5, dummy_w, None, parts.add_bf16, parts.add_bias,
-                               parts.slot, parts.delta, want_z=True)
+                               parts.slot, parts.delta, want_z=True, deferred=parts.deferred)
     return z
 
 
 def head(parts, norm, linear, packed=None):
     if packed is not None:
+        if parts.deferred is not None:
+            parts = Parts(materialize(parts))
         logits, _ = ops.ln_mean_head_varlen(parts.base, packed, norm.weight, norm.bias, norm.eps, linear.weight, linear.bias,
                                             parts.add_bf16, parts.add_bias, parts.slot, parts.delta)
         return logits
@@ -274,7 +277,7 @@
         from . import autograd as SA
         return SA.head_train(materialize(parts), norm, linear)
     logits, _, _ = ops.ln_mean_head(parts.base, norm.weight, norm.bias, norm.eps, linear.weight, linear.bias,
-                                    parts.add_bf16, parts.add_bias, parts.slot, parts.delta)
+                                    parts.add_bf16, parts.add_bias, parts.slot, parts.delta, deferred=parts.deferred)
     return logits
 
 
@@ -487,6 +490,13 @@
     return F.linear(x, lin.weight, lin.bias)
 
 
+def _ffn_out_hl(hid3, w2, b2, x2, deferred_ok):
+    if deferred_ok and ops.GEMM_HL_DEFERRED and ops.GEMM_HL_SPLITK \
+            and ops.gemm_hl_deferred_ws_bytes(hid3.shape[0], w2.shape[0], hid3.shape[1] // 2):
+        return ops.gemm_hl_deferred(hid3, w2, b2, resid=x2)
+    return ops.gemm_hl(hid3, w2, b2, resid=x2), None
+
+
 def encoder_layer(x2, sel, layer, need_attn, precision, packed=None, ragged=None, last=False):
     if packed is None and torch.is_grad_enabled() and (x2.requires_grad or any(p.requires_grad for p in layer.parameters())):
         from . import autograd as SA
@@ -587,14 +597,14 @@
             ops.layernorm_rows_hl_patch_(xn3, sel, xs, delta, eps=n1.eps)
             hid3 = ops.gemm_hl(xn3, fhf["w1"], fhf["b1"], ff.activation_name, hl_out=True)
             del xn3
-            z = ops.gemm_hl(hid3, fh["w2"], fw["b2"], resid=x2)
+            z, zk = _ffn_out_hl(hid3, fh["w2"], fw["b2"], x2, last and packed is None)
         elif hl:
             if x_sel is None:
                 x_sel = xs + delta
             yn3 = ops.layernorm_rows_hl(x2, n1.weight, n1.bias, n1.eps, slot=slot, patch_rows=x_sel)
             hid3 = ops.gemm_hl(yn3, fh["w1"], fw["b1"], ff.activation_name, hl_out=True)
             del yn3
-            z = ops.gemm_hl(hid3, fh["w2"], fw["b2"], resid=x2)
+            z, zk = _ffn_out_hl(hid3, fh["w2"], fw["b2"], x2, last and packed is None)
         else:
             if x_sel is None:
                 x_sel = xs + delta
@@ -602,9 +612,10 @@
             hid3 = ops.gemm_x3(yn3, fw["w1"], fw["b1"], ff.activation_name, split3=True)
             del yn3
             z = ops.gemm_x3(hid3, fw["w2"], fw["b2"], out_dtype=torch.float32, resid=x2)
+            zk = None
         del hid3
         if last:
-            return Parts(z, slot=slot, delta=delta), (attn.unsqueeze(0) if attn is not None else None)
+            return Parts(z, slot=slot, delta=delta, deferred=zk), (attn.unsqueeze(0) if attn is not None else None)
         ops.scatter_add_rows_(z, sel, delta)
         return Parts(z), (attn.unsqueeze(0) if attn is not None else None)
 
diff --git a/snuffy_amd/ops.py b/snuffy_amd/ops.py
--- a/snuffy_amd/ops.py
+++ b/snuffy_amd/ops.py
@@ -430,7 +430,7 @@
 
 
 def ln_mean_head(z, gamma, beta, eps, w_head, b_head, add_bf16=None, add_bias=None, slot=None, delta_rows=None,
-                 want_z=False):
+                 want_z=False, deferred=None):
     z = _req(z, torch.float32, "z", 2)
     n, d = z.shape
     if add_bf16 is not None:
@@ -452,6 +452,14 @@
     pooled = torch.empty(d, dtype=torch.float32, device=z.device)
     wsb = lib.snf_ln_mean_head_workspace_bytes(d)
     ws = _ws(wsb, z.device)
+    if deferred is not None:
+        if tuple(deferred.tile_map.shape) != ((n + 255) // 256, (d + 255) // 256):
+            raise ValueError("ln_mean_head: deferred part of a %s-tile result with z %s" % (tuple(deferred.tile_map.shape), (n, d)))
+        check(lib.snf_ln_mean_head_deferred_f32(_p(z), n, d, _p(deferred.slabs), _p(deferred.tile_map), deferred.tile_map.shape[1],
+                                                _p(add_bf16), _p(add_bias), _p(slot), _p(delta_rows), _p(z_out), _p(gamma), _p(beta),
+                                                float(eps), _p(w_head), _p(b_head), c, _p(logits), _p(pooled), _p(ws), wsb, _stream()),
+              "snf_ln_mean_head_deferred_f32")
+        return logits, pooled, z_out
     check(lib.snf_ln_mean_head_f32(_p(z), n, d, _p(add_bf16), _p(add_bias), _p(slot), _p(delta_rows), _p(z_out),
                                    _p(gamma), _p(beta), float(eps), _p(w_head), _p(b_head), c, _p(logits), _p(pooled),
                                    _p(ws), wsb, _stream()), "snf_ln_mean_head_f32")
@@ -1460,6 +1468,63 @@
 
 
 GEMM_HL_SPLITK = True
+GEMM_HL_DEFERRED = True
+
+
+class DeferredK:
+
+    __slots__ = ("slabs", "tile_map", "ws")
+
+    def __init__(self, slabs, tile_map, ws):
+        self.slabs, self.tile_map, self.ws = slabs, tile_map, ws
+
+    def add_to(self, z):
+        z = z.clone()
+        for tm, tn in self.tile_map.nonzero().tolist():
+            blk = z[256 * tm:256 * (tm + 1), 256 * tn:256 * (tn + 1)]
+            blk += self.slabs[int(self.tile_map[tm, tn]) - 1, :blk.shape[0], :blk.shape[1]]
+        return z
+
+
+def gemm_hl_deferred_ws_bytes(m, n, k):
+    return int(_ffi.load().snf_gemm_hl_deferred_ws_bytes(m, n, k, None))
+
+
+def gemm_hl_deferred(a_hl, w_hl, bias=None, resid=None, workspace=None):
+    if a_hl.dtype != torch.bfloat16 or w_hl.dtype != torch.bfloat16:
+        raise TypeError("gemm_hl_deferred: operands must be bfloat16 hl images")
+    a_hl = _rows16(a_hl, "a_hl")
+    w_hl = _rows16(w_hl, "w_hl")
+    m, k2 = a_hl.shape
+    n = w_hl.shape[0]
+    if w_hl.shape[1] != k2 or k2 % 64:
+        raise ValueError("gemm_hl_deferred: images are %s and %s" % (tuple(a_hl.shape), tuple(w_hl.shape)))
+    if bias is not None:
+        bias = _req(bias, torch.float32, "bias", 1)
+    ldr = 0
+    if resid is not None:
+        if resid.dtype != torch.float32 or tuple(resid.shape) != (m, n):
+            raise ValueError("gemm_hl_deferred: resid needs an fp32 [m, n] tensor")
+        resid = _rows16(resid, "resid")
+        ldr = resid.stride(0)
+    lib = _ffi.load()
+    off = ctypes.c_size_t(0)
+    ws_bytes = int(lib.snf_gemm_hl_deferred_ws_bytes(m, n, k2 // 2, ctypes.byref(off)))
+    if not ws_bytes:
+        raise ValueError("gemm_hl_deferred: m=%d n=%d k=%d has no split last round" % (m, n, k2 // 2))
+    ws = workspace
+    if ws is None:
+        ws = torch.empty(ws_bytes, dtype=torch.uint8, device=a_hl.device)
+    elif ws.dtype != torch.uint8 or ws.dim() != 1 or not ws.is_contiguous() or ws.numel() < ws_bytes or ws.device != a_hl.device:
+        raise ValueError("gemm_hl_deferred: workspace must be a contiguous uint8 tensor of >= %d bytes on %s" % (ws_bytes, a_hl.device))
+    out = torch.empty(m, n, dtype=torch.float32, device=a_hl.device)
+    check(lib.snf_gemm_hl_deferred_f32(_p(a_hl), a_hl.stride(0), _p(w_hl), w_hl.stride(0), _p(bias), _p(resid), ldr, m, n, k2 // 2,
+                                       ACT_CODES["none"], _p(out), out.stride(0), DT_F32, _p(ws), ws_bytes, _stream()),
+          "snf_gemm_hl_deferred_f32")
+    tm, tn = (m + 255) // 256, (n + 255) // 256
+    tile_map = ws[:4 * tm * tn].view(torch.int32).view(tm, tn)
+    slabs = ws[off.value:ws_bytes].view(torch.float32).view(-1, 256, 256)
+    return out, DeferredK(slabs, tile_map, ws)
 
 
 def _hl_workspace(device, nbytes):
diff --git a/snuffy_amd/snuffy.py b/snuffy_amd/snuffy.py
--- a/snuffy_amd/snuffy.py
+++ b/snuffy_amd/snuffy.py
@@ -293,7 +293,7 @@
     def _weights_signature(self):
         plist = list(self.parameters())
         knobs = tuple((l.big_lambda, l.random_patch_share) for l in self.b_classifier.encoder.layers)
-        knobs += (SF.FP32_GEMM, SF.FP32_ATTENTION, SF.X3_HL_ATTENTION, SF.X3_HL_KPFRAG, SF.X3_HL_KPFRAG_GATHER, SF.FP32_SHARED_NORM, ops.GEMM_HL_SPLITK,
+        knobs += (SF.FP32_GEMM, SF.FP32_ATTENTION, SF.X3_HL_ATTENTION, SF.X3_HL_KPFRAG, SF.X3_HL_KPFRAG_GATHER, SF.FP32_SHARED_NORM, ops.GEMM_HL_SPLITK, ops.GEMM_HL_DEFERRED,
                   SF.BF16_DEEP_STACKS, self.b_classifier.cfg.sampler)
         return tuple(SF.param_key(p) for p in plist), knobs
 
```

After: 898.1 slides/s, median of 6. 1.3% higher.
